# mit-han-lab/distrifuser

Hardware: NVIDIA H100
Metric: SDXL 50-step latency (ms/image) (lower is better)
Workload: dtype f16

## Files before the change

distrifuser_b200/_lib.py:

```python
from __future__ import annotations

import ctypes as C
import os

HERE = os.path.dirname(os.path.abspath(__file__))
LIB_PATH = os.environ.get("DF_LIB_PATH") or os.path.join(HERE, "libdistrifuser_b200.so")

NBANKS = 3
MAX_WORLD = 8
IPC_HANDLE_BYTES = 64
TENSORMAP_BYTES = 128
ZERO_CONV_MAX_PROBLEMS = 13

EXPORTS = (
    "df_last_error", "df_version", "df_device_sm_count", "df_symm_alloc", "df_symm_open", "df_symm_close",
    "df_symm_free", "df_step_begin", "df_slot_publish", "df_slot_wait", "df_groupnorm_scratch_bytes",
    "df_groupnorm_fwd", "df_groupnorm_halo_fwd", "df_groupnorm_fwd_weighted", "df_groupnorm_halo_fwd_weighted", "df_halo_push",
    "df_halo_assemble", "df_attn_make_kvmaps", "df_attn_workspace_bytes", "df_attn_fwd", "df_attn_make_kvmaps_ragged",
    "df_attn_workspace_bytes_ragged", "df_attn_fwd_ragged",
    "df_output_gather", "df_output_gather_2d", "df_geglu", "df_add_layernorm", "df_bias_residual_add", "df_linear_supported", "df_linear_geglu_block", "df_linear_fwd",
    "df_controlnet_zero_convs",
)


class DfComm(C.Structure):
    _fields_ = [("base", C.c_void_p * MAX_WORLD), ("flags", C.c_void_p * MAX_WORLD), ("clock", C.c_void_p),
                ("tickets", C.c_void_p), ("bank_stride", C.c_uint64), ("spin_timeout_ns", C.c_uint64), ("world", C.c_int32),
                ("rank", C.c_int32)]


_lib = None


def lib():
    global _lib
    if _lib is None:
        if not os.path.exists(LIB_PATH):
            raise RuntimeError(
                f"{LIB_PATH} is missing: build it with `python -m distrifuser_b200.build` "
                "(distrifuser_b200 has no fallback path; the CUDA extension is the product)")
        L = C.CDLL(LIB_PATH)
        vp, u64, i32, u32, i64, f32 = C.c_void_p, C.c_uint64, C.c_int, C.c_uint32, C.c_int64, C.c_float
        L.df_last_error.restype = C.c_char_p
        L.df_version.restype = i32
        L.df_device_sm_count.argtypes = [C.POINTER(i32)]
        L.df_symm_alloc.argtypes = [C.c_size_t, C.POINTER(vp), vp]
        L.df_symm_open.argtypes = [vp, C.POINTER(vp)]
        L.df_symm_close.argtypes = [vp]
        L.df_symm_free.argtypes = [vp]
        L.df_step_begin.argtypes = [vp, i32, vp]
        L.df_slot_publish.argtypes = [DfComm, vp, u64, u64, u64, u64, u64, i32, u32, i32, vp]
        L.df_slot_wait.argtypes = [DfComm, i32, u32, vp]
        L.df_groupnorm_scratch_bytes.argtypes = [i32, i32, i32, i32, i32]
        L.df_groupnorm_scratch_bytes.restype = C.c_size_t
        L.df_groupnorm_fwd.argtypes = [DfComm, vp, vp, i64, vp, vp, vp, i32, i32, i32, i32, i32, f32, i32, i32, i32, i32, i32,
                                       u64, u64, u32, vp, vp]
        L.df_groupnorm_halo_fwd.argtypes = [DfComm, vp, vp, i64, vp, vp, vp, i32, i32, i32, i32, i32, f32, i32, i32, i32, i32, i32,
                                            u64, u64, u32, vp, i32, u64, u64, i32, i32, i32, i32, vp]
        i32p = C.POINTER(C.c_int32)
        L.df_groupnorm_fwd_weighted.argtypes = [DfComm, vp, vp, i64, vp, vp, vp, i32, i32, i32, i32, i32, f32, i32, i32, i32, i32,
                                                i32, u64, u64, u32, i32p, vp, vp]
        L.df_groupnorm_halo_fwd_weighted.argtypes = [DfComm, vp, vp, i64, vp, vp, vp, i32, i32, i32, i32, i32, f32, i32, i32, i32,
                                                     i32, i32, u64, u64, u32, i32p, vp, i32, u64, u64, i32, i32, i32, i32, vp]
        L.df_attn_make_kvmaps_ragged.argtypes = [DfComm, u64, u64, i32, i32p, i32, i32, vp, vp]
        L.df_attn_workspace_bytes_ragged.argtypes = [i32, i32, i32p, i32, i32, i32]
        L.df_attn_workspace_bytes_ragged.restype = C.c_size_t
        L.df_attn_fwd_ragged.argtypes = [DfComm, vp, vp, vp, vp, i32, i32, i32p, i32, i32, i64, i64, i64, i32, i32, i32p, i32,
                                         i32, f32, vp, C.c_size_t, vp]
        L.df_halo_push.argtypes = [DfComm, vp, i32, i32, i32, i32, i32, u64, u64, i32, i32, vp]
        L.df_halo_assemble.argtypes = [DfComm, vp, vp, i32, i32, i32, i32, i32, u64, u64, i32, i32, i32, vp]
        L.df_attn_make_kvmaps.argtypes = [DfComm, u64, u64, i32, i32, i32, i32, vp, vp]
        L.df_attn_workspace_bytes.argtypes = [i32, i32, i32, i32, i32, i32]
        L.df_attn_workspace_bytes.restype = C.c_size_t
        L.df_attn_fwd.argtypes = [DfComm, vp, vp, vp, vp, i32, i32, i32, i32, i32, i64, i64, i64, i32, i32,
                                  C.POINTER(C.c_int32), i32, i32, f32, vp, C.c_size_t, vp]
        L.df_geglu.argtypes = [vp, vp, i64, i32, i64, i64, vp]
        L.df_add_layernorm.argtypes = [vp, vp, vp, vp, vp, vp, i64, i32, f32, vp]
        L.df_bias_residual_add.argtypes = [vp, vp, vp, vp, i64, i32, vp]
        L.df_linear_supported.argtypes = [i64, i32, i32, i32]
        L.df_linear_geglu_block.argtypes = [i64, i32, i32]
        L.df_linear_fwd.argtypes = [DfComm, vp, vp, vp, vp, vp, i64, i32, i32, i64, i64, i64, i64, i32, i32, i32, i32, i32, u32, u64,
                                    u64, i32, vp]
        L.df_controlnet_zero_convs.argtypes = [i32, C.POINTER(vp), C.POINTER(vp), C.POINTER(vp), C.POINTER(vp),
                                               C.POINTER(i64), C.POINTER(C.c_int32), C.POINTER(C.c_int32), vp, i32, vp]
        L.df_output_gather.argtypes = [DfComm, vp, vp, i32, i32, i32, i32, i32, i32, i32, i32, i32, u64, vp]
        L.df_output_gather_2d.argtypes = [DfComm, vp, vp, i32, i32, i32, i32, i32, i32, i32, i32, i32, i32, i32, u64, vp]
        for name in EXPORTS:
            getattr(L, name)
        _lib = L
    return _lib


KERNELS_PER_CALL = {"df_groupnorm_fwd": 1, "df_groupnorm_halo_fwd": 1, "df_attn_fwd": 1, "df_groupnorm_fwd_weighted": 1,
                    "df_groupnorm_halo_fwd_weighted": 1, "df_attn_fwd_ragged": 1, "df_halo_push": 1, "df_halo_assemble": 1,
                    "df_slot_publish": 1, "df_slot_wait": 1, "df_step_begin": 1, "df_output_gather": 2, "df_output_gather_2d": 2, "df_geglu": 1, "df_add_layernorm": 1, "df_bias_residual_add": 1,
                    "df_linear_fwd": 1, "df_controlnet_zero_convs": 1}
LAUNCHES = {"total": 0}
PROFILE = None


def check(rc: int, what: str = ""):
    LAUNCHES["total"] += KERNELS_PER_CALL.get(what, 0)
    if rc != 0:
        raise RuntimeError(f"distrifuser_b200 {what} failed ({rc}): {lib().df_last_error().decode()}")


def int32_array(values) -> C.Array:
    values = list(values)
    assert len(values) <= MAX_WORLD
    return (C.c_int32 * MAX_WORLD)(*values)


def null_comm() -> DfComm:
    c = DfComm()
    c.world, c.rank, c.bank_stride = 1, 0, 0
    return c
```

distrifuser_b200/csrc/linear.cu:

```cuda
#include <math.h>
#include <string.h>

#include "tc_ptx.cuh"

using namespace df;
using namespace df::tc;

namespace {

constexpr int BM = 128;
constexpr int BK = 64;
constexpr int NCONSUMER_WARPS = 8;
constexpr int NCONSUMERS = 32 * NCONSUMER_WARPS;
constexpr int NTHREADS = NCONSUMERS + 128;
constexpr int NEPILOGUE = 96;
constexpr int NTHREADS_ZC = NCONSUMERS + 32;
constexpr int CONSUMER_REGS = 208, WG2_REGS = 88;
constexpr uint32_t A_BYTES = BM * BK * 2;

template <int BN> struct Stages { static constexpr int value = BN == 256 ? 3 : 5; };

template <int BN>
struct __align__(1024) SmemT {
  __half a[Stages<BN>::value][BM * BK];
  __half b[Stages<BN>::value][BN * BK];
  uint64_t full[Stages<BN>::value], empty[Stages<BN>::value];
};

template <int BN> __host__ __device__ constexpr int stage_pitch() { return BN + 8; }

template <int BN>
struct __align__(1024) LinearSmem {
  SmemT<BN> ring;
  __half stg[BM * stage_pitch<BN>()];
  uint64_t stg_full, stg_empty;
};

enum { EPI_PLAIN = 0, EPI_GEGLU = 1 };

struct LinearArgs {
  const __half* bias;
  const __half* residual;
  __half* out;
  int64_t M;
  int N, K;
  int64_t ldr, ldo;
  int tiles_m, tiles_n;
  int publish;
  int pub_col0, pub_cols;
  int idx;
  uint32_t peer_mask;
  uint64_t tensor_off, slot_bytes;
  df_comm_t comm;
};

__device__ __forceinline__ float gelu_erf(float x) {
  const float z = fabsf(x) * 0.70710678118654752f;
  const float t = __fdividef(1.f, fmaf(0.3275911f, z, 1.f));
  float p = fmaf(1.061405429f, t, -1.453152027f);
  p = fmaf(p, t, 1.421413741f);
  p = fmaf(p, t, -0.284496736f);
  p = fmaf(p, t, 0.254829592f);
  const float e = p * t * __expf(-z * z);
  const float phi = x >= 0.f ? 1.f - 0.5f * e : 0.5f * e;
  return x * phi;
}

__device__ __forceinline__ float2 ld_h2f(const __half* p) { return __half22float2(*reinterpret_cast<const __half2*>(p)); }

__device__ __forceinline__ void stmatrix_x4(uint32_t addr, uint32_t r0, uint32_t r1, uint32_t r2, uint32_t r3) {
  asm volatile("stmatrix.sync.aligned.m8n8.x4.shared.b16 [%0], {%1, %2, %3, %4};" ::"r"(addr), "r"(r0), "r"(r1), "r"(r2), "r"(r3)
               : "memory");
}

union H8 {
  uint4 u;
  __half2 h[4];
};

template <int BN>
__device__ __forceinline__ void wgmma_tile(float* acc, uint64_t a_desc, uint64_t b_desc, uint32_t accumulate) {
  if constexpr (BN == 256) wgmma_ss_n256(acc, a_desc, b_desc, accumulate);
  else wgmma_ss_n160(acc, a_desc, b_desc, accumulate);
}

template <int BN>
__device__ __forceinline__ void load_tile(SmemT<BN>& sm, const void* tm_a, const void* tm_w, int tm, int tn, int kblocks,
                                          uint32_t& stage, uint32_t& phase) {
  constexpr int STAGES = Stages<BN>::value;
  constexpr uint32_t B_BYTES = BN * BK * 2;
  for (int kb = 0; kb < kblocks; ++kb) {
    mbar_wait(&sm.empty[stage], phase ^ 1u);
    mbar_expect_tx(&sm.full[stage], A_BYTES + B_BYTES);
    tma_load_2d(sm.a[stage], tm_a, &sm.full[stage], kb * BK, tm * BM);
    tma_load_2d(sm.b[stage], tm_w, &sm.full[stage], kb * BK, tn * BN);
    if (++stage == STAGES) { stage = 0; phase ^= 1u; }
  }
}

template <int BN>
__device__ __forceinline__ void mma_tile(SmemT<BN>& sm, float* acc, int wg, int lane, int kblocks, uint32_t& stage,
                                         uint32_t& phase) {
  constexpr int STAGES = Stages<BN>::value;
  fence_regs<BN / 2>(acc);
  uint32_t prev = 0;
  for (int kb = 0; kb < kblocks; ++kb) {
    mbar_wait(&sm.full[stage], phase);
    const uint32_t a_addr = smem_u32(sm.a[stage]) + wg * 64 * 128, b_addr = smem_u32(sm.b[stage]);
    wgmma_fence();
#pragma unroll
    for (int kk = 0; kk < BK / 16; ++kk)
      wgmma_tile<BN>(acc, smem_desc(a_addr + kk * 32, 16, 1024), smem_desc(b_addr + kk * 32, 16, 1024), (kb | kk) > 0);
    wgmma_commit();
    wgmma_wait<1>();
    if (kb > 0 && lane == 0) mbar_arrive(&sm.empty[prev]);
    prev = stage;
    if (++stage == STAGES) { stage = 0; phase ^= 1u; }
  }
  wgmma_wait<0>();
  fence_regs<BN / 2>(acc);
  if (lane == 0) mbar_arrive(&sm.empty[prev]);
}

template <int EPI, int BN>
__global__ void __launch_bounds__(NTHREADS, 1)
linear_kernel(const __grid_constant__ CUtensorMap tm_a, const __grid_constant__ CUtensorMap tm_w, LinearArgs p) {
  static_assert(BN % 32 == 0 && BN <= 256 && (BN * BK * 2) % 1024 == 0, "tile shape");
  constexpr int STAGES = Stages<BN>::value;
  constexpr int SP = stage_pitch<BN>();
  using Smem = LinearSmem<BN>;
  extern __shared__ __align__(1024) uint8_t smem_raw[];
  Smem& sm = *reinterpret_cast<Smem*>(smem_raw);
  if ((smem_u32(smem_raw) & 1023u) != 0) __trap();
  const int warp = threadIdx.x >> 5, lane = threadIdx.x & 31;
  const int ntiles = p.tiles_m * p.tiles_n;
  const int kblocks = p.K / BK;

  if (threadIdx.x == 0) {
    for (int s = 0; s < STAGES; ++s) { mbar_init(&sm.ring.full[s], 1); mbar_init(&sm.ring.empty[s], NCONSUMER_WARPS); }
    mbar_init(&sm.stg_full, NCONSUMERS);
    mbar_init(&sm.stg_empty, NEPILOGUE);
    asm volatile("fence.mbarrier_init.release.cluster;" ::: "memory");
  }
  __syncthreads();

  if (warp < NCONSUMER_WARPS) {
    setmaxnreg_inc<CONSUMER_REGS>();
    const int wg = warp >> 2;
    const int c4 = lane & 3;
    const int mrow = wg * 64 + (warp & 3) * 16 + ((lane >> 3) & 1) * 8 + (lane & 7);
    const uint32_t st_addr = smem_u32(sm.stg) + (uint32_t)(mrow * SP + (lane >> 4) * 8) * 2u;
    uint32_t stage = 0, phase = 0, sphase = 0;
    float acc[BN / 2];
    for (int tile = blockIdx.x; tile < ntiles; tile += gridDim.x) {
      const int tn = tile / p.tiles_m;
      __half2 bias2[BN / 8];
#pragma unroll
      for (int i = 0; i < BN / 8; ++i) {
        const int col = tn * BN + 8 * i + 2 * c4;
        bias2[i] = p.bias && col < p.N ? *reinterpret_cast<const __half2*>(p.bias + col) : __float2half2_rn(0.f);
      }
      mma_tile<BN>(sm.ring, acc, wg, lane, kblocks, stage, phase);
      mbar_wait(&sm.stg_empty, sphase ^ 1u);
#pragma unroll
      for (int j = 0; j < BN / 16; ++j) {
        uint32_t r[4];
#pragma unroll
        for (int q = 0; q < 2; ++q) {
          const int i = 2 * j + q;
          const float2 bb = __half22float2(bias2[i]);
          r[2 * q] = pack_h2(acc[4 * i] + bb.x, acc[4 * i + 1] + bb.y);
          r[2 * q + 1] = pack_h2(acc[4 * i + 2] + bb.x, acc[4 * i + 3] + bb.y);
        }
        stmatrix_x4(st_addr + j * 32, r[0], r[1], r[2], r[3]);
      }
      mbar_arrive(&sm.stg_full);
      sphase ^= 1u;
    }
  } else {
    setmaxnreg_dec<WG2_REGS>();
    if (warp == NCONSUMER_WARPS) {
      if (lane == 0) {
        prefetch_tmap(&tm_a);
        prefetch_tmap(&tm_w);
        uint32_t stage = 0, phase = 0;
        for (int tile = blockIdx.x; tile < ntiles; tile += gridDim.x)
          load_tile<BN>(sm.ring, &tm_a, &tm_w, tile % p.tiles_m, tile / p.tiles_m, kblocks, stage, phase);
      }
    } else {
      const int et = threadIdx.x - (NCONSUMERS + 32);
      uint32_t pub_epoch = 0;
      if (p.publish) pub_epoch = p.comm.clock[0];
      uint32_t sphase = 0;
      for (int tile = blockIdx.x; tile < ntiles; tile += gridDim.x) {
        const int tm = tile % p.tiles_m, tn = tile / p.tiles_m;
        mbar_wait(&sm.stg_full, sphase);
        if (EPI == EPI_GEGLU) {
          constexpr int CH = BN / 16;
          for (int v = et; v < BM * CH; v += NEPILOGUE) {
            const int r = v / CH, c = v % CH;
            const int64_t grow = (int64_t)tm * BM + r;
            if (grow >= p.M) continue;
            H8 hv, gv, o;
            hv.u = *reinterpret_cast<const uint4*>(sm.stg + r * SP + 8 * c);
            gv.u = *reinterpret_cast<const uint4*>(sm.stg + r * SP + 8 * (c + CH));
#pragma unroll
            for (int k = 0; k < 4; ++k) {
              const float2 hf = __half22float2(hv.h[k]), gf = __half22float2(gv.h[k]);
              o.h[k] = __floats2half2_rn(hf.x * gelu_erf(gf.x), hf.y * gelu_erf(gf.y));
            }
            *reinterpret_cast<uint4*>(p.out + grow * p.ldo + tn * (BN / 2) + 8 * c) = o.u;
          }
        } else {
          constexpr int CH = BN / 8;
#pragma unroll 4
          for (int v = et; v < BM * CH; v += NEPILOGUE) {
            const int r = v / CH, c = v % CH;
            const int64_t grow = (int64_t)tm * BM + r;
            const int col = tn * BN + 8 * c;
            if (grow >= p.M || col >= p.N) continue;
            H8 o;
            o.u = *reinterpret_cast<const uint4*>(sm.stg + r * SP + 8 * c);
            if (p.residual) {
              H8 rv;
              rv.u = __ldg(reinterpret_cast<const uint4*>(p.residual + grow * p.ldr + col));
#pragma unroll
              for (int k = 0; k < 4; ++k) o.h[k] = __hadd2(o.h[k], rv.h[k]);
            }
            *reinterpret_cast<uint4*>(p.out + grow * p.ldo + col) = o.u;
            if (p.publish && col >= p.pub_col0) {
              const uint64_t off = slot_offset(p.comm, pub_epoch, p.tensor_off, p.slot_bytes, p.comm.rank) +
                                   ((uint64_t)grow * p.pub_cols + (col - p.pub_col0)) * 2;
              for (int q = 0; q < p.comm.world; ++q)
                if (p.peer_mask >> q & 1) *reinterpret_cast<uint4*>((char*)p.comm.base[q] + off) = o.u;
            }
          }
        }
        mbar_arrive(&sm.stg_empty);
        sphase ^= 1u;
      }
    }
  }
  if (p.publish) signal_when_last(p.comm, &p.comm.tickets[p.idx], gridDim.x, p.idx, p.peer_mask, p.comm.clock[0]);
}

int make_map2d(CUtensorMap* m, const void* base, int64_t rows, int K, int64_t pitch, int box_rows) {
  EncodeTiledFn enc = tensor_map_encoder();
  DF_REQUIRE(enc != nullptr, "cuTensorMapEncodeTiled is not available from this driver");
  cuuint64_t dims[2] = {(cuuint64_t)K, (cuuint64_t)rows};
  cuuint64_t strides[1] = {(cuuint64_t)pitch * 2};
  cuuint32_t box[2] = {BK, (cuuint32_t)box_rows};
  cuuint32_t estr[2] = {1, 1};
  CUresult r = enc(m, CU_TENSOR_MAP_DATA_TYPE_FLOAT16, 2, const_cast<void*>(base), dims, strides, box, estr,
                   CU_TENSOR_MAP_INTERLEAVE_NONE, CU_TENSOR_MAP_SWIZZLE_128B, CU_TENSOR_MAP_L2_PROMOTION_L2_256B,
                   CU_TENSOR_MAP_FLOAT_OOB_FILL_NONE);
  DF_REQUIRE(r == CUDA_SUCCESS, "cuTensorMapEncodeTiled failed (%d): base=%p rows=%lld K=%d pitch=%lld", (int)r, base,
             (long long)rows, K, (long long)pitch);
  return 0;
}

template <int EPI, int BN>
int launch_linear(const CUtensorMap& ta, const CUtensorMap& tw, const LinearArgs& args, int ctas, cudaStream_t st) {
  static bool attr_set = false;
  if (!attr_set) {
    DF_CHECK_CUDA(cudaFuncSetAttribute(linear_kernel<EPI, BN>, cudaFuncAttributeMaxDynamicSharedMemorySize, (int)sizeof(LinearSmem<BN>)));
    attr_set = true;
  }
  linear_kernel<EPI, BN><<<ctas, NTHREADS, sizeof(LinearSmem<BN>), st>>>(ta, tw, args);
  DF_CHECK_LAUNCH();
  return 0;
}

double tile_cost(int64_t M, int N, int bn, int ctas_avail) {
  const long long tm = (M + BM - 1) / BM, tn = (N + bn - 1) / bn, tiles = tm * tn;
  const long long rounds = (tiles + ctas_avail - 1) / ctas_avail;
  return (double)rounds * (bn + 64);
}

}

namespace {
int pick_bn(int64_t M, int N, int epilogue, int cap) {
  const bool ok160 = epilogue == EPI_PLAIN || N % 160 == 0, ok256 = epilogue == EPI_PLAIN || N % 256 == 0;
  if (!ok256) return ok160 ? 160 : 0;
  if (ok160 && tile_cost(M, N, 160, cap) < 0.97 * tile_cost(M, N, 256, cap)) return 160;
  return 256;
}
}

extern "C" int df_linear_supported(int64_t M, int N, int K, int epilogue) {
  if (M < 1 || N < 8 || N % 8 != 0 || K < BK || K % BK != 0) return 0;
  if (epilogue == EPI_GEGLU && pick_bn(M, N, epilogue, sm_count()) == 0) return 0;
  return 1;
}

extern "C" int df_linear_geglu_block(int64_t M, int N, int K) {
  (void)K;
  const int bn = pick_bn(M, N, EPI_GEGLU, sm_count());
  return bn / 2;
}

extern "C" int df_linear_fwd(df_comm_t comm, const void* a, const void* w, const void* bias, const void* residual, void* out,
                             int64_t M, int N, int K, int64_t lda, int64_t ldw, int64_t ldr, int64_t ldo, int epilogue,
                             int geglu_block, int publish, int pub_col0, int idx, uint32_t peer_mask, uint64_t tensor_off,
                             uint64_t slot_bytes, int max_ctas, void* stream) {
  DF_REQUIRE(epilogue == EPI_PLAIN || epilogue == EPI_GEGLU, "df_linear_fwd: unknown epilogue %d", epilogue);
  DF_REQUIRE(df_linear_supported(M, N, K, epilogue), "df_linear_fwd: unsupported shape M=%lld N=%d K=%d (N %% 8, K %% 64%s)",
             (long long)M, N, K, epilogue == EPI_GEGLU ? ", GEGLU: N % 256" : "");
  DF_REQUIRE(((uintptr_t)a % 16) == 0 && ((uintptr_t)w % 16) == 0 && ((uintptr_t)out % 16) == 0 && ((uintptr_t)bias % 16) == 0 &&
                 ((uintptr_t)residual % 16) == 0 && lda % 8 == 0 && ldw % 8 == 0 && ldo % 8 == 0 && ldr % 8 == 0,
             "df_linear_fwd: operands must be 16-byte aligned with pitches multiple of 8");
  DF_REQUIRE(!(publish && epilogue != EPI_PLAIN), "df_linear_fwd: publication is a plain-epilogue feature");
  LinearArgs args;
  memset(&args, 0, sizeof(args));
  args.bias = (const __half*)bias; args.residual = (const __half*)residual; args.out = (__half*)out;
  args.M = M; args.N = N; args.K = K; args.ldr = ldr; args.ldo = ldo;
  const int sms = sm_count();
  const int cap = max_ctas > 0 ? max_ctas : sms;
  int bn = pick_bn(M, N, epilogue, epilogue == EPI_GEGLU ? sms : cap);
  if (epilogue == EPI_GEGLU && geglu_block > 0) {
    DF_REQUIRE(geglu_block == 80 || geglu_block == 128, "df_linear_fwd: geglu_block must be 80 or 128");
    bn = 2 * geglu_block;
    DF_REQUIRE(N % bn == 0, "df_linear_fwd: interleave block %d does not tile N=%d", geglu_block, N);
  }
  args.tiles_m = (int)((M + BM - 1) / BM);
  args.tiles_n = (N + bn - 1) / bn;
  args.publish = publish && peer_mask != 0;
  args.comm = comm;
  if (args.publish) {
    DF_REQUIRE(pub_col0 >= 0 && pub_col0 < N && pub_col0 % 8 == 0, "df_linear_fwd: bad pub_col0");
    DF_REQUIRE(tensor_off % 16 == 0 && slot_bytes % 16 == 0, "df_linear_fwd: slots must be 16-byte aligned");
    args.pub_col0 = pub_col0; args.pub_cols = N - pub_col0; args.idx = idx; args.peer_mask = peer_mask;
    args.tensor_off = tensor_off; args.slot_bytes = slot_bytes;
    DF_REQUIRE((uint64_t)M * args.pub_cols * 2 <= slot_bytes, "df_linear_fwd: published columns larger than the slot");
  }
  int ctas = args.tiles_m * args.tiles_n;
  if (ctas > cap) ctas = cap;
  if (ctas < 1) ctas = 1;
  CUtensorMap ta, tw;
  if (int rc = make_map2d(&ta, a, M, K, lda, BM)) return rc;
  if (int rc = make_map2d(&tw, w, N, K, ldw, bn)) return rc;
  cudaStream_t st = (cudaStream_t)stream;
  if (epilogue == EPI_GEGLU) {
    if (bn == 160) return launch_linear<EPI_GEGLU, 160>(ta, tw, args, ctas, st);
    return launch_linear<EPI_GEGLU, 256>(ta, tw, args, ctas, st);
  }
  if (bn == 160) return launch_linear<EPI_PLAIN, 160>(ta, tw, args, ctas, st);
  return launch_linear<EPI_PLAIN, 256>(ta, tw, args, ctas, st);
}

namespace {
constexpr int ZC_BN = 160;

struct ZeroConvProblem {
  const __half* bias;
  __half* out;
  int M, N, tiles_m, tile0, kblocks;
};

struct ZeroConvArgs {
  CUtensorMap a[DF_ZERO_CONV_MAX_PROBLEMS], w[DF_ZERO_CONV_MAX_PROBLEMS];
  ZeroConvProblem p[DF_ZERO_CONV_MAX_PROBLEMS];
  const float* scale;
  int nproblems, ntiles;
};
static_assert(sizeof(ZeroConvArgs) <= 4096, "the problem list must fit the 4 KiB kernel parameter space");

__device__ __forceinline__ int zc_problem(const ZeroConvArgs& z, int tile) {
  int q = 0;
  while (q + 1 < z.nproblems && tile >= z.p[q + 1].tile0) ++q;
  return q;
}

__global__ void __launch_bounds__(NTHREADS_ZC, 1) zero_conv_kernel(const __grid_constant__ ZeroConvArgs z) {
  constexpr int BN = ZC_BN;
  constexpr int STAGES = Stages<BN>::value;
  using Smem = SmemT<BN>;
  extern __shared__ __align__(1024) uint8_t smem_raw[];
  Smem& sm = *reinterpret_cast<Smem*>(smem_raw);
  if ((smem_u32(smem_raw) & 1023u) != 0) __trap();
  const int warp = threadIdx.x >> 5, lane = threadIdx.x & 31;

  if (threadIdx.x == 0) {
    for (int s = 0; s < STAGES; ++s) { mbar_init(&sm.full[s], 1); mbar_init(&sm.empty[s], NCONSUMER_WARPS); }
    asm volatile("fence.mbarrier_init.release.cluster;" ::: "memory");
  }
  __syncthreads();

  if (warp == NCONSUMER_WARPS) {
    if (lane == 0) {
      uint32_t stage = 0, phase = 0;
      for (int tile = blockIdx.x; tile < z.ntiles; tile += gridDim.x) {
        const int q = zc_problem(z, tile);
        const ZeroConvProblem& p = z.p[q];
        const int t = tile - p.tile0;
        load_tile<BN>(sm, &z.a[q], &z.w[q], t % p.tiles_m, t / p.tiles_m, p.kblocks, stage, phase);
      }
    }
  } else {
    const int wg = warp >> 2;
    const int c4 = lane & 3;
    const int rloc = wg * 64 + (warp & 3) * 16 + (lane >> 2);
    const float scale = *z.scale;
    uint32_t stage = 0, phase = 0;
    float acc[BN / 2];
    for (int tile = blockIdx.x; tile < z.ntiles; tile += gridDim.x) {
      const ZeroConvProblem& p = z.p[zc_problem(z, tile)];
      const int t = tile - p.tile0;
      const int tm = t % p.tiles_m, tn = t / p.tiles_m;
      mma_tile<BN>(sm, acc, wg, lane, p.kblocks, stage, phase);
#pragma unroll
      for (int h = 0; h < 2; ++h) {
        const int64_t grow = (int64_t)tm * BM + rloc + 8 * h;
        if (grow >= p.M) continue;
        const int col0 = tn * BN;
        __half* dst = p.out + grow * p.N + col0;
#pragma unroll
        for (int i = 0; i < BN / 8; ++i) {
          const int c = 8 * i + 2 * c4;
          const int col = col0 + c;
          if (col >= p.N) continue;
          float2 f = make_float2(acc[4 * i + 2 * h], acc[4 * i + 2 * h + 1]);
          if (p.bias) { const float2 bb = ld_h2f(p.bias + col); f.x += bb.x; f.y += bb.y; }
          const float2 r = __half22float2(__floats2half2_rn(f.x, f.y));
          *reinterpret_cast<__half2*>(dst + c) = __floats2half2_rn(r.x * scale, r.y * scale);
        }
      }
    }
  }
}
}

extern "C" int df_controlnet_zero_convs(int nproblems, const void* const* x_host, const void* const* w_host,
                                        const void* const* bias_host, void* const* out_host, const int64_t* m_host,
                                        const int32_t* n_host, const int32_t* k_host, const float* scale, int max_ctas,
                                        void* stream) {
  DF_REQUIRE(nproblems >= 1 && nproblems <= DF_ZERO_CONV_MAX_PROBLEMS, "df_controlnet_zero_convs: %d problems (1..%d)",
             nproblems, DF_ZERO_CONV_MAX_PROBLEMS);
  DF_REQUIRE(x_host && w_host && out_host && m_host && n_host && k_host && scale, "df_controlnet_zero_convs: null argument");
  DF_REQUIRE(((uintptr_t)scale % 4) == 0, "df_controlnet_zero_convs: scale must be a 4-byte aligned fp32");
  ZeroConvArgs z;
  memset(&z, 0, sizeof(z));
  int ntiles = 0;
  for (int i = 0; i < nproblems; ++i) {
    const int64_t M = m_host[i];
    const int N = n_host[i], K = k_host[i];
    const void* bias = bias_host ? bias_host[i] : nullptr;
    DF_REQUIRE(M >= 1 && M <= INT32_MAX && N >= 8 && N % 8 == 0 && K >= 8 && K % 8 == 0,
               "df_controlnet_zero_convs: problem %d has unsupported shape M=%lld N=%d K=%d (N %% 8, K %% 8)", i,
               (long long)M, N, K);
    DF_REQUIRE(x_host[i] && w_host[i] && out_host[i] && ((uintptr_t)x_host[i] % 16) == 0 &&
                   ((uintptr_t)w_host[i] % 16) == 0 && ((uintptr_t)out_host[i] % 16) == 0 && ((uintptr_t)bias % 16) == 0,
               "df_controlnet_zero_convs: problem %d: operands must be non-null and 16-byte aligned", i);
    if (int rc = make_map2d(&z.a[i], x_host[i], M, K, K, BM)) return rc;
    if (int rc = make_map2d(&z.w[i], w_host[i], N, K, K, ZC_BN)) return rc;
    ZeroConvProblem& p = z.p[i];
    p.bias = (const __half*)bias; p.out = (__half*)out_host[i];
    p.M = (int)M; p.N = N; p.kblocks = (K + BK - 1) / BK;
    p.tiles_m = (int)((M + BM - 1) / BM);
    p.tile0 = ntiles;
    const int64_t t = (int64_t)p.tiles_m * ((N + ZC_BN - 1) / ZC_BN);
    DF_REQUIRE(ntiles + t <= INT32_MAX, "df_controlnet_zero_convs: too many tiles");
    ntiles += (int)t;
  }
  z.scale = scale; z.nproblems = nproblems; z.ntiles = ntiles;
  const int cap = max_ctas > 0 ? max_ctas : sm_count();
  const int ctas = ntiles < cap ? ntiles : cap;
  static bool attr_set = false;
  if (!attr_set) {
    DF_CHECK_CUDA(cudaFuncSetAttribute(zero_conv_kernel, cudaFuncAttributeMaxDynamicSharedMemorySize, (int)sizeof(SmemT<ZC_BN>)));
    attr_set = true;
  }
  zero_conv_kernel<<<ctas, NTHREADS_ZC, sizeof(SmemT<ZC_BN>), (cudaStream_t)stream>>>(z);
  DF_CHECK_LAUNCH();
  return 0;
}
```

distrifuser_b200/csrc/tc_ptx.cuh:

```cuda
#pragma once
#include <cuda.h>

#include "common.cuh"

namespace df {
namespace tc {

__device__ __forceinline__ uint32_t smem_u32(const void* p) { return (uint32_t)__cvta_generic_to_shared(p); }

__device__ __forceinline__ void mbar_init(uint64_t* bar, uint32_t count) {
  asm volatile("mbarrier.init.shared::cta.b64 [%0], %1;" ::"r"(smem_u32(bar)), "r"(count));
}
__device__ __forceinline__ void mbar_expect_tx(uint64_t* bar, uint32_t bytes) {
  asm volatile("mbarrier.arrive.expect_tx.shared::cta.b64 _, [%0], %1;" ::"r"(smem_u32(bar)), "r"(bytes) : "memory");
}
__device__ __forceinline__ void mbar_arrive(uint32_t bar_addr) {
  asm volatile("mbarrier.arrive.shared::cta.b64 _, [%0];" ::"r"(bar_addr) : "memory");
}
__device__ __forceinline__ void mbar_arrive(uint64_t* bar) { mbar_arrive(smem_u32(bar)); }
constexpr uint32_t kTryWaitHintNs = 200000u;
__device__ __forceinline__ bool mbar_try(uint32_t bar_addr, uint32_t parity) {
  uint32_t ok;
  asm volatile(
      "{\n\t.reg .pred p;\n\t"
      "mbarrier.try_wait.parity.shared::cta.b64 p, [%1], %2, %3;\n\t"
      "selp.u32 %0, 1, 0, p;\n\t}"
      : "=r"(ok)
      : "r"(bar_addr), "r"(parity), "r"(kTryWaitHintNs)
      : "memory");
  return ok != 0;
}
__device__ __forceinline__ bool mbar_try(uint64_t* bar, uint32_t parity) { return mbar_try(smem_u32(bar), parity); }
__device__ __forceinline__ void mbar_wait(uint32_t bar, uint32_t parity) {
  if (mbar_try(bar, parity)) return;
  uint32_t polls = 0;
  uint64_t t0 = 0;
  while (!mbar_try(bar, parity)) {
    if ((++polls & 0x3FFu) == 0) {
      const uint64_t now = globaltimer_ns();
      if (t0 == 0) t0 = now;
      else if (now - t0 > 10000000000ull) {
#ifdef DF_MBAR_DEBUG
        printf("distrifuser_b200: mbarrier timeout (block %d,%d,%d thread %d bar@%u parity %u)\n", blockIdx.x, blockIdx.y, blockIdx.z,
               threadIdx.x, bar, parity);
#endif
        __trap();
      }
    }
  }
}

__device__ __forceinline__ void mbar_wait(uint64_t* bar, uint32_t parity) { mbar_wait(smem_u32(bar), parity); }

__device__ __forceinline__ void tma_load_4d(void* dst, const void* tmap, uint64_t* bar, int c0, int c1, int c2, int c3) {
  asm volatile(
      "cp.async.bulk.tensor.4d.shared::cluster.global.mbarrier::complete_tx::bytes [%0], [%1, {%3, %4, %5, %6}], [%2];"
      ::"r"(smem_u32(dst)), "l"((uint64_t)tmap), "r"(smem_u32(bar)), "r"(c0), "r"(c1), "r"(c2), "r"(c3)
      : "memory");
}
__device__ __forceinline__ void tma_load_2d(void* dst, const void* tmap, uint64_t* bar, int c0, int c1) {
  asm volatile(
      "cp.async.bulk.tensor.2d.shared::cluster.global.mbarrier::complete_tx::bytes [%0], [%1, {%3, %4}], [%2];"
      ::"r"(smem_u32(dst)), "l"((uint64_t)tmap), "r"(smem_u32(bar)), "r"(c0), "r"(c1)
      : "memory");
}
__device__ __forceinline__ void prefetch_tmap(const void* tmap) {
  asm volatile("prefetch.tensormap [%0];" ::"l"((uint64_t)tmap) : "memory");
}

__device__ __forceinline__ uint64_t smem_desc(uint32_t addr, uint32_t lbo_bytes, uint32_t sbo_bytes) {
  return (uint64_t)((addr & 0x3FFFFu) >> 4) | ((uint64_t)((lbo_bytes >> 4) & 0x3FFFu) << 16) |
         ((uint64_t)((sbo_bytes >> 4) & 0x3FFFu) << 32) | (1ull << 62);
}
__device__ __forceinline__ void wgmma_fence() { asm volatile("wgmma.fence.sync.aligned;" ::: "memory"); }
__device__ __forceinline__ void wgmma_commit() { asm volatile("wgmma.commit_group.sync.aligned;" ::: "memory"); }
template <int N>
__device__ __forceinline__ void wgmma_wait() { asm volatile("wgmma.wait_group.sync.aligned %0;" ::"n"(N) : "memory"); }
template <int N>
__device__ __forceinline__ void setmaxnreg_dec() { asm volatile("setmaxnreg.dec.sync.aligned.u32 %0;" ::"n"(N)); }
template <int N>
__device__ __forceinline__ void setmaxnreg_inc() { asm volatile("setmaxnreg.inc.sync.aligned.u32 %0;" ::"n"(N)); }
template <int ID, int COUNT>
__device__ __forceinline__ void named_bar_sync() { asm volatile("bar.sync %0, %1;" ::"n"(ID), "n"(COUNT) : "memory"); }
template <int ID, int COUNT>
__device__ __forceinline__ void named_bar_arrive() { asm volatile("bar.arrive %0, %1;" ::"n"(ID), "n"(COUNT) : "memory"); }
template <int N>
__device__ __forceinline__ void fence_regs(float* d) {
#pragma unroll
  for (int i = 0; i < N; ++i) asm volatile("" : "+f"(d[i])::"memory");
}

__device__ __forceinline__ void wgmma_ss_n64(float* d, uint64_t a_desc, uint64_t b_desc, uint32_t accumulate) {
  asm volatile(
      "{\n\t.reg .pred p;\n\tsetp.ne.b32 p, %34, 0;\n\t"
      "wgmma.mma_async.sync.aligned.m64n64k16.f32.f16.f16 {%0, %1, %2, %3, %4, %5, %6, %7, %8, %9, %10, %11, %12, %13, %14, %15, %16, %17, %18, %19, %20, %21, %22, %23, %24, %25, %26, %27, %28, %29, %30, %31}, %32, %33, p, 1, 1, 0, 0;\n\t}"
      : "+f"(d[0]), "+f"(d[1]), "+f"(d[2]), "+f"(d[3]), "+f"(d[4]), "+f"(d[5]), "+f"(d[6]), "+f"(d[7]), "+f"(d[8]), "+f"(d[9]), "+f"(d[10]), "+f"(d[11]), "+f"(d[12]), "+f"(d[13]), "+f"(d[14]), "+f"(d[15]), "+f"(d[16]), "+f"(d[17]), "+f"(d[18]), "+f"(d[19]), "+f"(d[20]), "+f"(d[21]), "+f"(d[22]), "+f"(d[23]), "+f"(d[24]), "+f"(d[25]), "+f"(d[26]), "+f"(d[27]), "+f"(d[28]), "+f"(d[29]), "+f"(d[30]), "+f"(d[31])
      : "l"(a_desc), "l"(b_desc), "r"(accumulate));
}
__device__ __forceinline__ void wgmma_ss_n128(float* d, uint64_t a_desc, uint64_t b_desc, uint32_t accumulate) {
  asm volatile(
      "{\n\t.reg .pred p;\n\tsetp.ne.b32 p, %66, 0;\n\t"
      "wgmma.mma_async.sync.aligned.m64n128k16.f32.f16.f16 {%0, %1, %2, %3, %4, %5, %6, %7, %8, %9, %10, %11, %12, %13, %14, %15, %16, %17, %18, %19, %20, %21, %22, %23, %24, %25, %26, %27, %28, %29, %30, %31, %32, %33, %34, %35, %36, %37, %38, %39, %40, %41, %42, %43, %44, %45, %46, %47, %48, %49, %50, %51, %52, %53, %54, %55, %56, %57, %58, %59, %60, %61, %62, %63}, %64, %65, p, 1, 1, 0, 0;\n\t}"
      : "+f"(d[0]), "+f"(d[1]), "+f"(d[2]), "+f"(d[3]), "+f"(d[4]), "+f"(d[5]), "+f"(d[6]), "+f"(d[7]), "+f"(d[8]), "+f"(d[9]), "+f"(d[10]), "+f"(d[11]), "+f"(d[12]), "+f"(d[13]), "+f"(d[14]), "+f"(d[15]), "+f"(d[16]), "+f"(d[17]), "+f"(d[18]), "+f"(d[19]), "+f"(d[20]), "+f"(d[21]), "+f"(d[22]), "+f"(d[23]), "+f"(d[24]), "+f"(d[25]), "+f"(d[26]), "+f"(d[27]), "+f"(d[28]), "+f"(d[29]), "+f"(d[30]), "+f"(d[31]), "+f"(d[32]), "+f"(d[33]), "+f"(d[34]), "+f"(d[35]), "+f"(d[36]), "+f"(d[37]), "+f"(d[38]), "+f"(d[39]), "+f"(d[40]), "+f"(d[41]), "+f"(d[42]), "+f"(d[43]), "+f"(d[44]), "+f"(d[45]), "+f"(d[46]), "+f"(d[47]), "+f"(d[48]), "+f"(d[49]), "+f"(d[50]), "+f"(d[51]), "+f"(d[52]), "+f"(d[53]), "+f"(d[54]), "+f"(d[55]), "+f"(d[56]), "+f"(d[57]), "+f"(d[58]), "+f"(d[59]), "+f"(d[60]), "+f"(d[61]), "+f"(d[62]), "+f"(d[63])
      : "l"(a_desc), "l"(b_desc), "r"(accumulate));
}

__device__ __forceinline__ void wgmma_ss_n160(float* d, uint64_t a_desc, uint64_t b_desc, uint32_t accumulate) {
  asm volatile(
      "{\n\t.reg .pred p;\n\tsetp.ne.b32 p, %82, 0;\n\t"
      "wgmma.mma_async.sync.aligned.m64n160k16.f32.f16.f16 {%0, %1, %2, %3, %4, %5, %6, %7, %8, %9, %10, %11, %12, %13, %14, %15, %16, %17, %18, %19, %20, %21, %22, %23, %24, %25, %26, %27, %28, %29, %30, %31, %32, %33, %34, %35, %36, %37, %38, %39, %40, %41, %42, %43, %44, %45, %46, %47, %48, %49, %50, %51, %52, %53, %54, %55, %56, %57, %58, %59, %60, %61, %62, %63, %64, %65, %66, %67, %68, %69, %70, %71, %72, %73, %74, %75, %76, %77, %78, %79}, %80, %81, p, 1, 1, 0, 0;\n\t}"
      : "+f"(d[0]), "+f"(d[1]), "+f"(d[2]), "+f"(d[3]), "+f"(d[4]), "+f"(d[5]), "+f"(d[6]), "+f"(d[7]), "+f"(d[8]), "+f"(d[9]), "+f"(d[10]), "+f"(d[11]), "+f"(d[12]), "+f"(d[13]), "+f"(d[14]), "+f"(d[15]), "+f"(d[16]), "+f"(d[17]), "+f"(d[18]), "+f"(d[19]), "+f"(d[20]), "+f"(d[21]), "+f"(d[22]), "+f"(d[23]), "+f"(d[24]), "+f"(d[25]), "+f"(d[26]), "+f"(d[27]), "+f"(d[28]), "+f"(d[29]), "+f"(d[30]), "+f"(d[31]), "+f"(d[32]), "+f"(d[33]), "+f"(d[34]), "+f"(d[35]), "+f"(d[36]), "+f"(d[37]), "+f"(d[38]), "+f"(d[39]), "+f"(d[40]), "+f"(d[41]), "+f"(d[42]), "+f"(d[43]), "+f"(d[44]), "+f"(d[45]), "+f"(d[46]), "+f"(d[47]), "+f"(d[48]), "+f"(d[49]), "+f"(d[50]), "+f"(d[51]), "+f"(d[52]), "+f"(d[53]), "+f"(d[54]), "+f"(d[55]), "+f"(d[56]), "+f"(d[57]), "+f"(d[58]), "+f"(d[59]), "+f"(d[60]), "+f"(d[61]), "+f"(d[62]), "+f"(d[63]), "+f"(d[64]), "+f"(d[65]), "+f"(d[66]), "+f"(d[67]), "+f"(d[68]), "+f"(d[69]), "+f"(d[70]), "+f"(d[71]), "+f"(d[72]), "+f"(d[73]), "+f"(d[74]), "+f"(d[75]), "+f"(d[76]), "+f"(d[77]), "+f"(d[78]), "+f"(d[79])
      : "l"(a_desc), "l"(b_desc), "r"(accumulate));
}

__device__ __forceinline__ void wgmma_ss_n256(float* d, uint64_t a_desc, uint64_t b_desc, uint32_t accumulate) {
  asm volatile(
      "{\n\t.reg .pred p;\n\tsetp.ne.b32 p, %130, 0;\n\t"
      "wgmma.mma_async.sync.aligned.m64n256k16.f32.f16.f16 {%0, %1, %2, %3, %4, %5, %6, %7, %8, %9, %10, %11, %12, %13, %14, %15, %16, %17, %18, %19, %20, %21, %22, %23, %24, %25, %26, %27, %28, %29, %30, %31, %32, %33, %34, %35, %36, %37, %38, %39, %40, %41, %42, %43, %44, %45, %46, %47, %48, %49, %50, %51, %52, %53, %54, %55, %56, %57, %58, %59, %60, %61, %62, %63, %64, %65, %66, %67, %68, %69, %70, %71, %72, %73, %74, %75, %76, %77, %78, %79, %80, %81, %82, %83, %84, %85, %86, %87, %88, %89, %90, %91, %92, %93, %94, %95, %96, %97, %98, %99, %100, %101, %102, %103, %104, %105, %106, %107, %108, %109, %110, %111, %112, %113, %114, %115, %116, %117, %118, %119, %120, %121, %122, %123, %124, %125, %126, %127}, %128, %129, p, 1, 1, 0, 0;\n\t}"
      : "+f"(d[0]), "+f"(d[1]), "+f"(d[2]), "+f"(d[3]), "+f"(d[4]), "+f"(d[5]), "+f"(d[6]), "+f"(d[7]), "+f"(d[8]), "+f"(d[9]), "+f"(d[10]), "+f"(d[11]), "+f"(d[12]), "+f"(d[13]), "+f"(d[14]), "+f"(d[15]), "+f"(d[16]), "+f"(d[17]), "+f"(d[18]), "+f"(d[19]), "+f"(d[20]), "+f"(d[21]), "+f"(d[22]), "+f"(d[23]), "+f"(d[24]), "+f"(d[25]), "+f"(d[26]), "+f"(d[27]), "+f"(d[28]), "+f"(d[29]), "+f"(d[30]), "+f"(d[31]), "+f"(d[32]), "+f"(d[33]), "+f"(d[34]), "+f"(d[35]), "+f"(d[36]), "+f"(d[37]), "+f"(d[38]), "+f"(d[39]), "+f"(d[40]), "+f"(d[41]), "+f"(d[42]), "+f"(d[43]), "+f"(d[44]), "+f"(d[45]), "+f"(d[46]), "+f"(d[47]), "+f"(d[48]), "+f"(d[49]), "+f"(d[50]), "+f"(d[51]), "+f"(d[52]), "+f"(d[53]), "+f"(d[54]), "+f"(d[55]), "+f"(d[56]), "+f"(d[57]), "+f"(d[58]), "+f"(d[59]), "+f"(d[60]), "+f"(d[61]), "+f"(d[62]), "+f"(d[63]), "+f"(d[64]), "+f"(d[65]), "+f"(d[66]), "+f"(d[67]), "+f"(d[68]), "+f"(d[69]), "+f"(d[70]), "+f"(d[71]), "+f"(d[72]), "+f"(d[73]), "+f"(d[74]), "+f"(d[75]), "+f"(d[76]), "+f"(d[77]), "+f"(d[78]), "+f"(d[79]), "+f"(d[80]), "+f"(d[81]), "+f"(d[82]), "+f"(d[83]), "+f"(d[84]), "+f"(d[85]), "+f"(d[86]), "+f"(d[87]), "+f"(d[88]), "+f"(d[89]), "+f"(d[90]), "+f"(d[91]), "+f"(d[92]), "+f"(d[93]), "+f"(d[94]), "+f"(d[95]), "+f"(d[96]), "+f"(d[97]), "+f"(d[98]), "+f"(d[99]), "+f"(d[100]), "+f"(d[101]), "+f"(d[102]), "+f"(d[103]), "+f"(d[104]), "+f"(d[105]), "+f"(d[106]), "+f"(d[107]), "+f"(d[108]), "+f"(d[109]), "+f"(d[110]), "+f"(d[111]), "+f"(d[112]), "+f"(d[113]), "+f"(d[114]), "+f"(d[115]), "+f"(d[116]), "+f"(d[117]), "+f"(d[118]), "+f"(d[119]), "+f"(d[120]), "+f"(d[121]), "+f"(d[122]), "+f"(d[123]), "+f"(d[124]), "+f"(d[125]), "+f"(d[126]), "+f"(d[127])
      : "l"(a_desc), "l"(b_desc), "r"(accumulate));
}

__device__ __forceinline__ void wgmma_rs_n64(float* d, const uint32_t* a, uint64_t b_desc, uint32_t accumulate) {
  asm volatile(
      "{\n\t.reg .pred p;\n\tsetp.ne.b32 p, %37, 0;\n\t"
      "wgmma.mma_async.sync.aligned.m64n64k16.f32.f16.f16 {%0, %1, %2, %3, %4, %5, %6, %7, %8, %9, %10, %11, %12, %13, %14, %15, %16, %17, %18, %19, %20, %21, %22, %23, %24, %25, %26, %27, %28, %29, %30, %31}, {%32, %33, %34, %35}, %36, p, 1, 1, 1;\n\t}"
      : "+f"(d[0]), "+f"(d[1]), "+f"(d[2]), "+f"(d[3]), "+f"(d[4]), "+f"(d[5]), "+f"(d[6]), "+f"(d[7]), "+f"(d[8]), "+f"(d[9]), "+f"(d[10]), "+f"(d[11]), "+f"(d[12]), "+f"(d[13]), "+f"(d[14]), "+f"(d[15]), "+f"(d[16]), "+f"(d[17]), "+f"(d[18]), "+f"(d[19]), "+f"(d[20]), "+f"(d[21]), "+f"(d[22]), "+f"(d[23]), "+f"(d[24]), "+f"(d[25]), "+f"(d[26]), "+f"(d[27]), "+f"(d[28]), "+f"(d[29]), "+f"(d[30]), "+f"(d[31])
      : "r"(a[0]), "r"(a[1]), "r"(a[2]), "r"(a[3]), "l"(b_desc), "r"(accumulate));
}


__device__ __forceinline__ float ex2(float x) {
  float y;
  asm("ex2.approx.ftz.f32 %0, %1;" : "=f"(y) : "f"(x));
  return y;
}
__device__ __forceinline__ float ex2_poly(float x) {
  x = fmaxf(x, -127.f);
  const float r = __fadd_rd(x, 12582912.f);
  const float f = x - (r - 12582912.f);
  float q = fmaf(f, 0.077119089663028717041015625f, 0.227564394474029541015625f);
  q = fmaf(q, f, 0.695146143436431884765625f);
  q = fmaf(q, f, 1.f);
  return __int_as_float(__float_as_int(q) + (__float_as_int(r) << 23));
}
__device__ __forceinline__ uint32_t pack_h2(float lo, float hi) {
  __half2 h = __floats2half2_rn(lo, hi);
  return *reinterpret_cast<uint32_t*>(&h);
}


}
}
```

distrifuser_b200/modules/pp/attn.py:

```python
import ctypes as C

import torch
from torch import nn
from torch.nn import functional as F

from ... import _lib
from ...utils import DistriConfig
from ..base_module import BaseModule, nvtx_range


_WORKSPACES: dict = {}


def _shared_workspace(device, nbytes: int) -> torch.Tensor:
    lst = _WORKSPACES.setdefault(device, [])
    if not lst or lst[-1].numel() < nbytes:
        if torch.cuda.is_current_stream_capturing():
            raise RuntimeError("attention workspace would grow during CUDA-graph capture; run one eager UNet call first")
        lst.append(torch.zeros(max(nbytes, 16 << 20), dtype=torch.uint8, device=device))
    return lst[-1]


class DistriAttentionPP(BaseModule):
    def __init__(self, module: nn.Module, distri_config: DistriConfig):
        super().__init__(module, distri_config)
        to_k, to_v = module.to_k, module.to_v
        assert isinstance(to_k, nn.Linear) and isinstance(to_v, nn.Linear)
        assert (to_k.bias is None) == (to_v.bias is None)
        assert to_k.weight.shape == to_v.weight.shape
        in_size, out_size = to_k.in_features, to_k.out_features
        to_kv = nn.Linear(in_size, out_size * 2, bias=to_k.bias is not None, device=to_k.weight.device,
                          dtype=to_k.weight.dtype)
        with torch.no_grad():
            to_kv.weight[:out_size].copy_(to_k.weight)
            to_kv.weight[out_size:].copy_(to_v.weight)
            if to_k.bias is not None:
                to_kv.bias[:out_size].copy_(to_k.bias)
                to_kv.bias[out_size:].copy_(to_v.bias)
        self.to_kv = to_kv
        self._kvmaps = None

    def _attend(self, q, kv_own, lens, own_seg, wait_flags, kind="self", scale=0.0, real_width=None):
        attn = self.module
        b, lq, Cq = q.shape
        heads = attn.heads
        d = Cq // heads
        out = torch.empty((b, lq, Cq), dtype=q.dtype, device=q.device)
        cm = self.comm_manager
        nseg = len(lens)
        if nseg > 1:
            comm, maps = cm.group, self._kvmaps.data_ptr()
        else:
            comm, maps = _lib.null_comm(), None
        seg_rank = (C.c_int32 * _lib.MAX_WORLD)(*range(_lib.MAX_WORLD))
        seg_len = _lib.int32_array(lens)
        L = _lib.lib()
        ws_bytes = L.df_attn_workspace_bytes_ragged(b, lq, seg_len, nseg, heads, d)
        ws = _shared_workspace(q.device, ws_bytes).data_ptr() if ws_bytes else None
        prof = _lib.PROFILE
        if prof is not None:
            e0, e1 = torch.cuda.Event(enable_timing=True), torch.cuda.Event(enable_timing=True)
            e0.record()
        _lib.check(L.df_attn_fwd_ragged(comm, q.data_ptr(), kv_own.data_ptr(), out.data_ptr(), maps, b, lq, seg_len,
                                        heads, d, q.stride(1), kv_own.stride(1), out.stride(1), nseg, own_seg,
                                        seg_rank, self.idx or 0, int(wait_flags), float(scale), ws, ws_bytes,
                                        torch.cuda.current_stream().cuda_stream), "df_attn_fwd_ragged")
        if prof is not None:
            e1.record()
            prof.append(dict(kernel="fmha_fwd_kernel", kind=kind,
                             flops=4.0 * b * lq * sum(lens) * (real_width or Cq),
                             bytes=2.0 * (2 * b * lq * Cq + b * sum(lens) * 2 * Cq),
                             shape=(b, lq, sum(lens), heads, d), start=e0, end=e1))
        return out

    def _project_out(self, hidden_states, residual, weight=None):
        from ... import ops
        attn = self.module
        hidden_states = ops.project("out", hidden_states, attn.to_out[0], weight)
        hidden_states = attn.to_out[1](hidden_states)
        if attn.residual_connection:
            hidden_states = hidden_states + residual
        if attn.rescale_output_factor != 1.0:
            hidden_states = hidden_states / attn.rescale_output_factor
        return hidden_states


class DistriCrossAttentionPP(DistriAttentionPP):
    def __init__(self, module: nn.Module, distri_config: DistriConfig):
        super().__init__(module, distri_config)
        self.kv_cache = None

    @nvtx_range("DistriCrossAttentionPP")
    def forward(self, hidden_states, encoder_hidden_states=None, scale: float = 1.0, *args, **kwargs):
        assert encoder_hidden_states is not None
        self._require_cuda_half(hidden_states, "DistriCrossAttentionPP")
        attn = self.module
        from ... import ops
        q = ops.project("qkv", hidden_states, attn.to_q)
        if self.counter == 0 or self.kv_cache is None:
            kv = self.to_kv(encoder_hidden_states)
            if self.kv_cache is not None and self.kv_cache.shape == kv.shape:
                self.kv_cache.copy_(kv)
            else:
                self.kv_cache = kv
        kv = self.kv_cache
        out = self._attend(q, kv, [kv.shape[1]], 0, False, kind="cross")
        out = self._project_out(out, hidden_states)
        self.counter += 1
        return out


class DistriSelfAttentionPP(DistriAttentionPP):
    def __init__(self, module: nn.Module, distri_config: DistriConfig):
        super().__init__(module, distri_config)
        self._w_qkv = None
        self._w_qkv_key = None
        self._w_out = None
        self._head_pad = 0

    def _qkv_weight(self, dtype):
        to_q, to_kv = self.module.to_q, self.to_kv
        if not (isinstance(to_q, nn.Linear) and to_q.bias is None and to_kv.bias is None and
                to_q.in_features == to_kv.in_features and to_q.out_features * 2 == to_kv.out_features and
                to_q.weight.dtype == dtype and to_kv.weight.dtype == dtype):
            return None
        wq, wkv, wo = to_q.weight, to_kv.weight, self.module.to_out[0].weight
        heads = self.module.heads
        d = to_q.out_features // heads
        pad = 64 if d < 64 else 0
        key = (wq._version, wkv._version, wo._version, wq.data_ptr(), wkv.data_ptr(), wo.data_ptr(), wq.device, dtype, pad)
        if key != self._w_qkv_key:
            if torch.cuda.is_current_stream_capturing():
                raise RuntimeError("DistriSelfAttentionPP: attention weights changed since the last eager call; run one "
                                   "eager UNet call (pipeline.prepare()) before capturing CUDA graphs")
            with torch.no_grad():
                if pad:
                    cin = wq.shape[1]
                    widen = lambda w: F.pad(w.detach().reshape(-1, heads, d, cin), (0, 0, 0, pad - d)).reshape(-1, cin)
                    self._w_qkv = torch.cat([widen(wq), widen(wkv)], 0).contiguous()
                    self._w_out = F.pad(wo.detach().reshape(wo.shape[0], heads, d), (0, pad - d)).reshape(wo.shape[0], heads * pad).contiguous()
                else:
                    self._w_qkv = torch.cat([wq.detach(), wkv.detach()], 0).contiguous()
                    self._w_out = None
            self._w_qkv_key = key
            self._head_pad = pad
        return self._w_qkv

    @nvtx_range("DistriSelfAttentionPP")
    def forward(self, hidden_states, encoder_hidden_states=None, scale: float = 1.0, *args, **kwargs):
        cfg = self.distri_config
        self._require_cuda_half(hidden_states, "DistriSelfAttentionPP")
        attn = self.module
        n, r = cfg.n_device_per_batch, cfg.split_idx()
        b, l, c = hidden_states.shape
        cm = self.comm_manager
        w_qkv = self._qkv_weight(hidden_states.dtype)
        heads = attn.heads
        d_real = c // heads
        padded = w_qkv is not None and self._head_pad != 0
        cs = heads * self._head_pad if padded else c
        lens = self.patch_rows(l) if n > 1 else [l]
        if n > 1 and self._recording() and self.idx is None:
            self.idx = cm.register_tensor((b, l, 2 * cs), hidden_states.dtype, layer_type="attn",
                                          slot_bytes=b * max(lens) * 2 * cs * hidden_states.element_size())
        live = n > 1 and self._bound()
        sync = live and (cfg.mode == "full_sync" or self._is_sync_step())
        ship = live and (sync or cfg.mode != "no_sync")
        published = False
        if w_qkv is not None:
            from ... import ops
            if not padded and ops.use_fused_linear("qkv") and ops.linear_supported(b * l, 3 * c, c):
                pub = (cm.group, c, self.idx, cm.peers_mask(), cm.tensor_off[self.idx], cm.slot_bytes[self.idx]) if ship else None
                qkv = ops.linear(hidden_states, w_qkv, publish=pub)
                published = ship
            else:
                qkv = F.linear(hidden_states, w_qkv)
            q, kv = qkv[..., :cs], qkv[..., cs:]
        else:
            q = attn.to_q(hidden_states)
            kv = self.to_kv(hidden_states)
        sm_scale = d_real ** -0.5 if padded else 0.0
        if not live:
            out = self._attend(q, kv, [l], 0, False, scale=sm_scale, real_width=c)
        else:
            if self._kvmaps is None:
                self._kvmaps = torch.empty(_lib.NBANKS * n * _lib.TENSORMAP_BYTES, dtype=torch.uint8, device=q.device)
                _lib.check(_lib.lib().df_attn_make_kvmaps_ragged(cm.group, cm.tensor_off[self.idx], cm.slot_bytes[self.idx], b,
                                                                 _lib.int32_array(lens), heads, cs // heads,
                                                                 self._kvmaps.data_ptr(), torch.cuda.current_stream().cuda_stream),
                           "df_attn_make_kvmaps_ragged")
            if ship and not published:
                cm.enqueue(self.idx, kv, async_stream=not sync)
            out = self._attend(q, kv, lens, r, True, scale=sm_scale, real_width=c)
        out = self._project_out(out, hidden_states, self._w_out if padded else None)
        self.counter += 1
        return out
```

distrifuser_b200/ops.py:

```python
import os as _os

import torch

from . import _lib


def geglu(y: torch.Tensor) -> torch.Tensor:
    assert y.is_cuda and y.dtype == torch.float16 and y.stride(-1) == 1
    cols = y.shape[-1] // 2
    y2 = y.reshape(-1, 2 * cols)
    out = torch.empty((*y.shape[:-1], cols), dtype=y.dtype, device=y.device)
    _lib.check(_lib.lib().df_geglu(y2.data_ptr(), out.data_ptr(), y2.shape[0], cols, y2.stride(0), cols,
                                   torch.cuda.current_stream().cuda_stream), "df_geglu")
    return out


def add_layernorm(x: torch.Tensor, r: torch.Tensor | None, norm: torch.nn.LayerNorm):
    assert x.is_cuda and x.dtype == torch.float16
    C = x.shape[-1]
    x = x.contiguous()
    y = torch.empty_like(x)
    if r is not None:
        r = r.contiguous()
        s = torch.empty_like(x)
    else:
        s = x
    _lib.check(_lib.lib().df_add_layernorm(x.data_ptr(), r.data_ptr() if r is not None else None,
                                           s.data_ptr() if r is not None else None, y.data_ptr(), norm.weight.data_ptr(),
                                           norm.bias.data_ptr(), x.numel() // C, C, float(norm.eps),
                                           torch.cuda.current_stream().cuda_stream), "df_add_layernorm")
    return s, y


def conv2d_bias_residual(x: torch.Tensor, conv: torch.nn.Conv2d, padding, residual: torch.Tensor | None = None,
                         bias: torch.Tensor | None = None, fold_bias: bool = False) -> torch.Tensor:
    import torch.nn.functional as F
    b = conv.bias if bias is None else bias
    ok = (x.is_cuda and x.dtype == torch.float16 and conv.out_channels % 8 == 0 and
          x.is_contiguous(memory_format=torch.channels_last))
    if not ok:
        out = F.conv2d(x, conv.weight, None if fold_bias else b, stride=conv.stride, padding=padding)
        return out if residual is None else residual + out
    out = F.conv2d(x, conv.weight, None, stride=conv.stride, padding=padding)
    if (b is None or fold_bias) and residual is None:
        return out
    if not out.is_contiguous(memory_format=torch.channels_last):
        out = out.contiguous(memory_format=torch.channels_last)
    if b is None or fold_bias:
        return residual + out
    if residual is not None:
        assert residual.shape == out.shape and residual.dtype == out.dtype
        if not residual.is_contiguous(memory_format=torch.channels_last):
            residual = residual.contiguous(memory_format=torch.channels_last)
    n, c, h, w = out.shape
    _lib.check(_lib.lib().df_bias_residual_add(out.data_ptr(), residual.data_ptr() if residual is not None else None,
                                               b.data_ptr(), out.data_ptr(), n * h * w, c,
                                               torch.cuda.current_stream().cuda_stream), "df_bias_residual_add")
    return out



_FUSED_LINEAR = set(_os.environ.get("DF_LINEAR", "geglu").replace("all", "geglu,qkv,out,ff2,proj").split(","))


def use_fused_linear(kind: str) -> bool:
    return kind in _FUSED_LINEAR


GEGLU_BLOCK = 128


def linear_supported(M: int, N: int, K: int, geglu: bool = False) -> bool:
    return bool(_lib.lib().df_linear_supported(M, N, K, 1 if geglu else 0))


def geglu_block(M: int, two_d: int, K: int) -> int:
    if not linear_supported(M, two_d, K, geglu=True):
        return 0
    return int(_lib.lib().df_linear_geglu_block(M, two_d, K))


def geglu_interleave(weight: torch.Tensor, bias: torch.Tensor | None, block: int = GEGLU_BLOCK):
    two_d, K = weight.shape
    D = two_d // 2
    assert D % block == 0
    w = torch.stack([weight[:D].reshape(D // block, block, K), weight[D:].reshape(D // block, block, K)], 1)
    w = w.reshape(two_d, K).contiguous()
    b = None
    if bias is not None:
        b = torch.stack([bias[:D].reshape(-1, block), bias[D:].reshape(-1, block)], 1).reshape(two_d).contiguous()
    return w, b


def linear(x: torch.Tensor, weight: torch.Tensor, bias: torch.Tensor | None = None, residual: torch.Tensor | None = None,
           out: torch.Tensor | None = None, publish=None) -> torch.Tensor:
    assert x.is_cuda and x.dtype == torch.float16 and weight.dtype == torch.float16 and x.stride(-1) == 1 and weight.stride(-1) == 1
    K = x.shape[-1]
    N = weight.shape[0]
    x2 = x.reshape(-1, K)
    M = x2.shape[0]
    if out is None:
        out = torch.empty((*x.shape[:-1], N), dtype=x.dtype, device=x.device)
    o2 = out.view(-1, N)
    r2 = residual.reshape(-1, N) if residual is not None else None
    if publish is not None:
        comm, pub_col0, idx, mask, off, sb = publish
    else:
        comm, pub_col0, idx, mask, off, sb = _lib.null_comm(), 0, 0, 0, 0, 0
    _lib.check(_lib.lib().df_linear_fwd(comm, x2.data_ptr(), weight.data_ptr(), bias.data_ptr() if bias is not None else None,
                                        r2.data_ptr() if r2 is not None else None, o2.data_ptr(), M, N, K, x2.stride(0),
                                        weight.stride(0), r2.stride(0) if r2 is not None else 0, o2.stride(0), 0, 0,
                                        int(publish is not None), pub_col0, idx, mask, off, sb, 0,
                                        torch.cuda.current_stream().cuda_stream), "df_linear_fwd")
    return out


def project(kind: str, x: torch.Tensor, lin: torch.nn.Linear, weight: torch.Tensor | None = None) -> torch.Tensor:
    w = lin.weight if weight is None else weight
    K = x.shape[-1]
    if (use_fused_linear(kind) and x.is_cuda and x.dtype == torch.float16 and w.dtype == torch.float16 and
            x.stride(-1) == 1 and w.stride(-1) == 1 and getattr(lin, "lora_layer", None) is None and
            linear_supported(x.numel() // K, w.shape[0], K)):
        return linear(x, w, lin.bias)
    if weight is None:
        return lin(x)
    import torch.nn.functional as F
    return F.linear(x, weight, lin.bias)


def linear_geglu(x: torch.Tensor, w_interleaved: torch.Tensor, b_interleaved: torch.Tensor | None, block: int = GEGLU_BLOCK) -> torch.Tensor:
    assert x.is_cuda and x.dtype == torch.float16 and x.stride(-1) == 1
    K = x.shape[-1]
    N = w_interleaved.shape[0]
    x2 = x.reshape(-1, K)
    out = torch.empty((*x.shape[:-1], N // 2), dtype=x.dtype, device=x.device)
    _lib.check(_lib.lib().df_linear_fwd(_lib.null_comm(), x2.data_ptr(), w_interleaved.data_ptr(),
                                        b_interleaved.data_ptr() if b_interleaved is not None else None, None, out.data_ptr(),
                                        x2.shape[0], N, K, x2.stride(0), w_interleaved.stride(0), 0, N // 2, 1, block, 0, 0, 0, 0, 0, 0, 0,
                                        torch.cuda.current_stream().cuda_stream), "df_linear_fwd")
    return out


def controlnet_zero_convs(xs, convs, scale: torch.Tensor) -> list[torch.Tensor]:
    import ctypes as C
    n = len(xs)
    assert len(convs) == n and scale.is_cuda and scale.dtype == torch.float32 and scale.numel() == 1
    outs, xp, wp, bp, op, ms, ns, ks = [], [], [], [], [], [], [], []
    for x, conv in zip(xs, convs):
        assert x.is_cuda and x.dtype == torch.float16 and tuple(conv.kernel_size) == (1, 1)
        x = x.contiguous(memory_format=torch.channels_last)
        b, k, h, w = x.shape
        out = torch.empty((b, conv.out_channels, h, w), dtype=x.dtype, device=x.device, memory_format=torch.channels_last)
        outs.append(out)
        xp.append(x.data_ptr()); wp.append(conv.weight.data_ptr()); op.append(out.data_ptr())
        bp.append(conv.bias.data_ptr() if conv.bias is not None else None)
        ms.append(b * h * w); ns.append(conv.out_channels); ks.append(k)
    ptrs = lambda v: (C.c_void_p * n)(*v)
    _lib.check(_lib.lib().df_controlnet_zero_convs(n, ptrs(xp), ptrs(wp), ptrs(bp), ptrs(op), (C.c_int64 * n)(*ms),
                                                   (C.c_int32 * n)(*ns), (C.c_int32 * n)(*ks), scale.data_ptr(), 0,
                                                   torch.cuda.current_stream().cuda_stream), "df_controlnet_zero_convs")
    return outs
```

include/distrifuser_b200.h:

```cpp
#ifndef DISTRIFUSER_B200_H
#define DISTRIFUSER_B200_H

#include <stddef.h>
#include <stdint.h>

#ifdef __cplusplus
extern "C" {
#endif

#define DF_NBANKS 3
#define DF_MAX_WORLD 8
#define DF_IPC_HANDLE_BYTES 64
#define DF_TENSORMAP_BYTES 128
#define DF_ZERO_CONV_MAX_PROBLEMS 13

const char* df_last_error(void);
int df_version(void);
int df_device_sm_count(int* out);

int df_symm_alloc(size_t bytes, void** dptr, void* ipc_handle_out_host );
int df_symm_open(const void* ipc_handle_host, void** peer_dptr);
int df_symm_close(void* peer_dptr);
int df_symm_free(void* dptr);

typedef struct {
  void* base[DF_MAX_WORLD];
  uint32_t* flags[DF_MAX_WORLD];
  uint32_t* clock;
  uint32_t* tickets;
  uint64_t bank_stride;
  uint64_t spin_timeout_ns;
  int32_t world;
  int32_t rank;
} df_comm_t;

int df_step_begin(uint32_t* clock, int kind, void* stream);

int df_slot_publish(df_comm_t comm, const void* src, uint64_t rows, uint64_t row_bytes, uint64_t src_pitch,
                    uint64_t tensor_off, uint64_t slot_bytes, int idx, uint32_t peer_mask, int num_ctas,
                    void* stream);

int df_slot_wait(df_comm_t comm, int idx, uint32_t src_mask, void* stream);

size_t df_groupnorm_scratch_bytes(int b, int groups, int h, int w, int C);
int df_groupnorm_fwd(df_comm_t comm, const void* x, const void* addend, int64_t addend_pitch, void* y, const void* gamma, const void* beta,
                     int b, int h, int w, int C, int groups, float eps, int mode, int bessel,
                     int neg_var_fallback, int fuse_silu, int idx, uint64_t tensor_off, uint64_t slot_bytes,
                     uint32_t group_mask, void* scratch, void* stream);

int df_groupnorm_halo_fwd(df_comm_t comm, const void* x, const void* addend, int64_t addend_pitch, void* y_padded, const void* gamma, const void* beta,
                          int b, int h, int w, int C, int groups, float eps, int mode, int bessel, int neg_var_fallback,
                          int fuse_silu, int idx, uint64_t tensor_off, uint64_t slot_bytes, uint32_t group_mask, void* scratch,
                          int halo_idx, uint64_t halo_off, uint64_t halo_slot_bytes, int up_rank, int down_rank, int push,
                          int wait_flags, void* stream);

int df_groupnorm_fwd_weighted(df_comm_t comm, const void* x, const void* addend, int64_t addend_pitch, void* y, const void* gamma,
                              const void* beta, int b, int h, int w, int C, int groups, float eps, int mode, int bessel,
                              int neg_var_fallback, int fuse_silu, int idx, uint64_t tensor_off, uint64_t slot_bytes,
                              uint32_t group_mask, const int32_t* src_weight_host , void* scratch, void* stream);
int df_groupnorm_halo_fwd_weighted(df_comm_t comm, const void* x, const void* addend, int64_t addend_pitch, void* y_padded,
                                   const void* gamma, const void* beta, int b, int h, int w, int C, int groups, float eps, int mode,
                                   int bessel, int neg_var_fallback, int fuse_silu, int idx, uint64_t tensor_off,
                                   uint64_t slot_bytes, uint32_t group_mask, const int32_t* src_weight_host ,
                                   void* scratch, int halo_idx, uint64_t halo_off, uint64_t halo_slot_bytes, int up_rank,
                                   int down_rank, int push, int wait_flags, void* stream);

int df_halo_push(df_comm_t comm, const void* x, int b, int h, int w, int C, int idx, uint64_t tensor_off,
                 uint64_t slot_bytes, int up_rank, int down_rank, void* stream);
int df_halo_assemble(df_comm_t comm, const void* x, void* xp, int b, int h, int w, int C, int idx,
                     uint64_t tensor_off, uint64_t slot_bytes, int up_rank, int down_rank, int wait_flags,
                     void* stream);

int df_attn_make_kvmaps(df_comm_t comm, uint64_t tensor_off, uint64_t slot_bytes, int b, int lseg, int heads,
                        int d, void* maps_out , void* stream);
size_t df_attn_workspace_bytes(int b, int lq, int lseg, int nseg, int heads, int d);
int df_attn_fwd(df_comm_t comm, const void* q, const void* kv_own, void* out, const void* kvmaps,
                int b, int lq, int lseg, int heads, int d, int64_t q_pitch, int64_t kv_pitch, int64_t o_pitch,
                int nseg, int own_seg, const int32_t* seg_rank_host, int idx, int wait_flags, float scale,
                void* workspace, size_t workspace_bytes, void* stream);
int df_attn_make_kvmaps_ragged(df_comm_t comm, uint64_t tensor_off, uint64_t slot_bytes, int b, const int32_t* seg_len_host,
                               int heads, int d, void* maps_out , void* stream);
size_t df_attn_workspace_bytes_ragged(int b, int lq, const int32_t* seg_len_host, int nseg, int heads, int d);
int df_attn_fwd_ragged(df_comm_t comm, const void* q, const void* kv_own, void* out, const void* kvmaps,
                       int b, int lq, const int32_t* seg_len_host, int heads, int d, int64_t q_pitch, int64_t kv_pitch,
                       int64_t o_pitch, int nseg, int own_seg, const int32_t* seg_rank_host, int idx, int wait_flags, float scale,
                       void* workspace, size_t workspace_bytes, void* stream);

int df_output_gather(df_comm_t comm, const void* strip, void* out, int B, int C, int H, int W, int bs, int hs,
                     int batch0, int row0, int idx, uint64_t tensor_off, void* stream);

int df_output_gather_2d(df_comm_t comm, const void* strip, void* out, int B, int C, int H, int W, int bs, int hs, int ws,
                        int batch0, int row0, int col0, int idx, uint64_t tensor_off, void* stream);

int df_geglu(const void* in, void* out, int64_t rows, int cols, int64_t in_pitch, int64_t out_pitch, void* stream);

int df_bias_residual_add(const void* a, const void* residual , const void* bias, void* out, int64_t rows, int C,
                         void* stream);

int df_add_layernorm(const void* x, const void* r, void* s_out, void* y, const void* gamma, const void* beta,
                     int64_t rows, int C, float eps, void* stream);

int df_linear_supported(int64_t M, int N, int K, int epilogue);
int df_linear_geglu_block(int64_t M, int N, int K);
int df_linear_fwd(df_comm_t comm, const void* a, const void* w, const void* bias, const void* residual, void* out,
                  int64_t M, int N, int K, int64_t lda, int64_t ldw, int64_t ldr, int64_t ldo, int epilogue,
                  int geglu_block, int publish, int pub_col0, int idx, uint32_t peer_mask, uint64_t tensor_off,
                  uint64_t slot_bytes, int max_ctas, void* stream);

int df_controlnet_zero_convs(int nproblems, const void* const* x_host, const void* const* w_host, const void* const* bias_host,
                             void* const* out_host, const int64_t* m_host, const int32_t* n_host, const int32_t* k_host,
                             const float* scale, int max_ctas, void* stream);

#ifdef __cplusplus
}
#endif
#endif
```

Before: 1521.

## Fuse cross-attention Q projection and softmax attention into the linear GEMM kernel

Adds a cross-attention epilogue to the warp-specialized linear kernel. After the Q projection tile is computed, the kernel adds the bias and, for each 64-wide head, runs QK^T, softmax and PV in registers against the cached text K/V (at most 80 tokens), with K/V loaded by TMA into the ring stages. This removes the separate Q projection kernel, the round trip of Q through global memory and the separate attention launch. In exchange it adds N=192/128 tile variants, higher register pressure, and a new code path limited to head_dim 64 and at most 80 KV tokens.

```diff
diff --git a/distrifuser_b200/_lib.py b/distrifuser_b200/_lib.py
--- a/distrifuser_b200/_lib.py
+++ b/distrifuser_b200/_lib.py
@@ -19,7 +19,7 @@
     "df_halo_assemble", "df_attn_make_kvmaps", "df_attn_workspace_bytes", "df_attn_fwd", "df_attn_make_kvmaps_ragged",
     "df_attn_workspace_bytes_ragged", "df_attn_fwd_ragged",
     "df_output_gather", "df_output_gather_2d", "df_geglu", "df_add_layernorm", "df_bias_residual_add", "df_linear_supported", "df_linear_geglu_block", "df_linear_fwd",
-    "df_controlnet_zero_convs",
+    "df_linear_cross_attn_supported", "df_linear_cross_attn_fwd", "df_controlnet_zero_convs",
 )
 
 
@@ -81,6 +81,8 @@
         L.df_linear_geglu_block.argtypes = [i64, i32, i32]
         L.df_linear_fwd.argtypes = [DfComm, vp, vp, vp, vp, vp, i64, i32, i32, i64, i64, i64, i64, i32, i32, i32, i32, i32, u32, u64,
                                     u64, i32, vp]
+        L.df_linear_cross_attn_supported.argtypes = [i32, i32, i32, i32, i32, i32]
+        L.df_linear_cross_attn_fwd.argtypes = [vp, vp, vp, vp, vp, i32, i32, i32, i32, i32, i32, i64, i64, f32, i32, vp]
         L.df_controlnet_zero_convs.argtypes = [i32, C.POINTER(vp), C.POINTER(vp), C.POINTER(vp), C.POINTER(vp),
                                                C.POINTER(i64), C.POINTER(C.c_int32), C.POINTER(C.c_int32), vp, i32, vp]
         L.df_output_gather.argtypes = [DfComm, vp, vp, i32, i32, i32, i32, i32, i32, i32, i32, i32, u64, vp]
@@ -94,7 +96,7 @@
 KERNELS_PER_CALL = {"df_groupnorm_fwd": 1, "df_groupnorm_halo_fwd": 1, "df_attn_fwd": 1, "df_groupnorm_fwd_weighted": 1,
                     "df_groupnorm_halo_fwd_weighted": 1, "df_attn_fwd_ragged": 1, "df_halo_push": 1, "df_halo_assemble": 1,
                     "df_slot_publish": 1, "df_slot_wait": 1, "df_step_begin": 1, "df_output_gather": 2, "df_output_gather_2d": 2, "df_geglu": 1, "df_add_layernorm": 1, "df_bias_residual_add": 1,
-                    "df_linear_fwd": 1, "df_controlnet_zero_convs": 1}
+                    "df_linear_fwd": 1, "df_linear_cross_attn_fwd": 1, "df_controlnet_zero_convs": 1}
 LAUNCHES = {"total": 0}
 PROFILE = None
 
diff --git a/distrifuser_b200/csrc/linear.cu b/distrifuser_b200/csrc/linear.cu
--- a/distrifuser_b200/csrc/linear.cu
+++ b/distrifuser_b200/csrc/linear.cu
@@ -18,7 +18,7 @@
 constexpr int CONSUMER_REGS = 208, WG2_REGS = 88;
 constexpr uint32_t A_BYTES = BM * BK * 2;
 
-template <int BN> struct Stages { static constexpr int value = BN == 256 ? 3 : 5; };
+template <int BN> struct Stages { static constexpr int value = BN == 256 ? 3 : BN == 192 ? 4 : 5; };
 
 template <int BN>
 struct __align__(1024) SmemT {
@@ -36,7 +36,11 @@
   uint64_t stg_full, stg_empty;
 };
 
-enum { EPI_PLAIN = 0, EPI_GEGLU = 1 };
+enum { EPI_PLAIN = 0, EPI_GEGLU = 1, EPI_CROSS = 2 };
+
+constexpr int HEAD_D = 64;
+constexpr int LKV_ROWS = 80;
+constexpr uint32_t KV_BYTES = LKV_ROWS * HEAD_D * 2;
 
 struct LinearArgs {
   const __half* bias;
@@ -52,6 +56,8 @@
   uint32_t peer_mask;
   uint64_t tensor_off, slot_bytes;
   df_comm_t comm;
+  int L, mt, lkv;
+  float scale_log2;
 };
 
 __device__ __forceinline__ float gelu_erf(float x) {
@@ -81,18 +87,21 @@
 template <int BN>
 __device__ __forceinline__ void wgmma_tile(float* acc, uint64_t a_desc, uint64_t b_desc, uint32_t accumulate) {
   if constexpr (BN == 256) wgmma_ss_n256(acc, a_desc, b_desc, accumulate);
-  else wgmma_ss_n160(acc, a_desc, b_desc, accumulate);
+  else if constexpr (BN == 192) wgmma_ss_n192(acc, a_desc, b_desc, accumulate);
+  else if constexpr (BN == 160) wgmma_ss_n160(acc, a_desc, b_desc, accumulate);
+  else wgmma_ss_n128(acc, a_desc, b_desc, accumulate);
 }
 
 template <int BN>
-__device__ __forceinline__ void load_tile(SmemT<BN>& sm, const void* tm_a, const void* tm_w, int tm, int tn, int kblocks,
-                                          uint32_t& stage, uint32_t& phase) {
+__device__ __forceinline__ void load_tile(SmemT<BN>& sm, const void* tm_a, const void* tm_w, int a_row, int a_bat, int tn,
+                                          int kblocks, uint32_t& stage, uint32_t& phase) {
   constexpr int STAGES = Stages<BN>::value;
   constexpr uint32_t B_BYTES = BN * BK * 2;
   for (int kb = 0; kb < kblocks; ++kb) {
     mbar_wait(&sm.empty[stage], phase ^ 1u);
     mbar_expect_tx(&sm.full[stage], A_BYTES + B_BYTES);
-    tma_load_2d(sm.a[stage], tm_a, &sm.full[stage], kb * BK, tm * BM);
+    if (a_bat < 0) tma_load_2d(sm.a[stage], tm_a, &sm.full[stage], kb * BK, a_row);
+    else tma_load_3d(sm.a[stage], tm_a, &sm.full[stage], kb * BK, a_row, a_bat);
     tma_load_2d(sm.b[stage], tm_w, &sm.full[stage], kb * BK, tn * BN);
     if (++stage == STAGES) { stage = 0; phase ^= 1u; }
   }
@@ -122,10 +131,115 @@
   if (lane == 0) mbar_arrive(&sm.empty[prev]);
 }
 
+template <int BN>
+__device__ __forceinline__ void cross_attend(SmemT<BN>& sm, float* acc, const __half2* bias2, uint32_t st_addr, int lane,
+                                             int lkv, float scale_log2, uint32_t& stage, uint32_t& phase) {
+  constexpr int STAGES = Stages<BN>::value;
+  constexpr int NH = BN / HEAD_D;
+  const int c4 = lane & 3;
+  uint32_t qf[BN / 4];
+#pragma unroll
+  for (int i = 0; i < BN / 8; ++i) {
+    const float2 bb = __half22float2(bias2[i]);
+    qf[2 * i] = pack_h2(acc[4 * i] + bb.x, acc[4 * i + 1] + bb.y);
+    qf[2 * i + 1] = pack_h2(acc[4 * i + 2] + bb.x, acc[4 * i + 3] + bb.y);
+  }
+  uint32_t hs[NH], hp[NH];
+#pragma unroll
+  for (int h = 0; h < NH; ++h) {
+    hs[h] = stage; hp[h] = phase;
+    if (++stage == STAGES) { stage = 0; phase ^= 1u; }
+  }
+  auto k_addr = [&](int h) { return BN == 256 ? smem_u32(sm.b[hs[h]]) : smem_u32(sm.a[hs[h]]); };
+  auto v_addr = [&](int h) { return BN == 256 ? smem_u32(sm.b[hs[h]]) + KV_BYTES : smem_u32(sm.b[hs[h]]); };
+  constexpr bool S_IN_ACC = LKV_ROWS <= BN / 2, O_IN_ACC = LKV_ROWS + HEAD_D / 2 <= BN / 2;
+  float s_own[S_IN_ACC ? 1 : LKV_ROWS], o_own[O_IN_ACC ? 1 : HEAD_D / 2];
+  float* const s_buf = S_IN_ACC ? acc : s_own;
+  float* s[2] = {s_buf, s_buf + LKV_ROWS / 2};
+  auto issue_s = [&](int h) {
+    mbar_wait(&sm.full[hs[h]], hp[h]);
+    wgmma_fence();
+#pragma unroll
+    for (int kk = 0; kk < HEAD_D / 16; ++kk)
+      wgmma_rs_n80(s[h & 1], qf + 16 * h + 4 * kk, smem_desc(k_addr(h) + kk * 32, 16, 1024), kk > 0);
+    wgmma_commit();
+  };
+  issue_s(0);
+#pragma unroll
+  for (int h = 0; h < NH; ++h) {
+    float* S = s[h & 1];
+    if (h + 1 < NH) {
+      issue_s(h + 1);
+      wgmma_wait<1>();
+    } else {
+      wgmma_wait<0>();
+    }
+    fence_regs<LKV_ROWS / 2>(S);
+    auto sv = [&](int i, int k) {
+      const float x = S[4 * i + k];
+      return 8 * i + 2 * c4 + (k & 1) >= lkv ? -INFINITY : x;
+    };
+    float mA0 = -INFINITY, mA1 = -INFINITY, mB0 = -INFINITY, mB1 = -INFINITY;
+#pragma unroll
+    for (int i = 0; i < LKV_ROWS / 8; i += 2) {
+      mA0 = fmaxf(mA0, fmaxf(sv(i, 0), sv(i, 1)));
+      mB0 = fmaxf(mB0, fmaxf(sv(i, 2), sv(i, 3)));
+      mA1 = fmaxf(mA1, fmaxf(sv(i + 1, 0), sv(i + 1, 1)));
+      mB1 = fmaxf(mB1, fmaxf(sv(i + 1, 2), sv(i + 1, 3)));
+    }
+    float mA = fmaxf(mA0, mA1), mB = fmaxf(mB0, mB1);
+    mA = fmaxf(mA, __shfl_xor_sync(0xffffffffu, mA, 1));
+    mB = fmaxf(mB, __shfl_xor_sync(0xffffffffu, mB, 1));
+    mA = fmaxf(mA, __shfl_xor_sync(0xffffffffu, mA, 2));
+    mB = fmaxf(mB, __shfl_xor_sync(0xffffffffu, mB, 2));
+    const float nA = -mA * scale_log2, nB = -mB * scale_log2;
+    float lA = 0.f, lB = 0.f;
+    uint32_t pk[LKV_ROWS / 4];
+#pragma unroll
+    for (int i = 0; i < LKV_ROWS / 8; ++i) {
+      const float p0 = ex2(fmaf(sv(i, 0), scale_log2, nA)), p1 = ex2(fmaf(sv(i, 1), scale_log2, nA));
+      const float p2 = ex2(fmaf(sv(i, 2), scale_log2, nB)), p3 = ex2(fmaf(sv(i, 3), scale_log2, nB));
+      lA += p0 + p1;
+      lB += p2 + p3;
+      pk[2 * i] = pack_h2(p0, p1);
+      pk[2 * i + 1] = pack_h2(p2, p3);
+    }
+    float* o = O_IN_ACC ? acc + LKV_ROWS : o_own;
+    wgmma_fence();
+#pragma unroll
+    for (int kk = 0; kk < LKV_ROWS / 16; ++kk)
+      wgmma_rs_n64(o, pk + 4 * kk, smem_desc(v_addr(h) + kk * 2048, KV_BYTES, 1024), kk > 0);
+    wgmma_commit();
+    lA += __shfl_xor_sync(0xffffffffu, lA, 1); lB += __shfl_xor_sync(0xffffffffu, lB, 1);
+    lA += __shfl_xor_sync(0xffffffffu, lA, 2); lB += __shfl_xor_sync(0xffffffffu, lB, 2);
+    const float invA = 1.f / lA, invB = 1.f / lB;
+    wgmma_wait<0>();
+    fence_regs<HEAD_D / 2>(o);
+    if (h + 1 < NH) fence_regs<LKV_ROWS / 2>(s[(h + 1) & 1]);
+    __syncwarp();
+    if (lane == 0) mbar_arrive(&sm.empty[hs[h]]);
+#pragma unroll
+    for (int j = 0; j < HEAD_D / 16; ++j) {
+      uint32_t r[4];
+#pragma unroll
+      for (int q = 0; q < 2; ++q) {
+        const int i = 2 * j + q;
+        r[2 * q] = pack_h2(o[4 * i] * invA, o[4 * i + 1] * invA);
+        r[2 * q + 1] = pack_h2(o[4 * i + 2] * invB, o[4 * i + 3] * invB);
+      }
+      stmatrix_x4(st_addr + (h * (HEAD_D / 16) + j) * 32, r[0], r[1], r[2], r[3]);
+    }
+  }
+}
+
 template <int EPI, int BN>
 __global__ void __launch_bounds__(NTHREADS, 1)
-linear_kernel(const __grid_constant__ CUtensorMap tm_a, const __grid_constant__ CUtensorMap tm_w, LinearArgs p) {
+linear_kernel(const __grid_constant__ CUtensorMap tm_a, const __grid_constant__ CUtensorMap tm_w,
+              const __grid_constant__ CUtensorMap tm_kv, LinearArgs p) {
   static_assert(BN % 32 == 0 && BN <= 256 && (BN * BK * 2) % 1024 == 0, "tile shape");
+  static_assert(EPI != EPI_CROSS || (BN % HEAD_D == 0 && (BN == 256 ? 2 * KV_BYTES <= BN * BK * 2
+                                                                    : KV_BYTES <= A_BYTES && KV_BYTES <= BN * BK * 2)),
+                "cross-attention: whole heads per tile, K and V of a head in one stage");
   constexpr int STAGES = Stages<BN>::value;
   constexpr int SP = stage_pitch<BN>();
   using Smem = LinearSmem<BN>;
@@ -162,17 +276,21 @@
       }
       mma_tile<BN>(sm.ring, acc, wg, lane, kblocks, stage, phase);
       mbar_wait(&sm.stg_empty, sphase ^ 1u);
-#pragma unroll
-      for (int j = 0; j < BN / 16; ++j) {
-        uint32_t r[4];
-#pragma unroll
-        for (int q = 0; q < 2; ++q) {
-          const int i = 2 * j + q;
-          const float2 bb = __half22float2(bias2[i]);
-          r[2 * q] = pack_h2(acc[4 * i] + bb.x, acc[4 * i + 1] + bb.y);
-          r[2 * q + 1] = pack_h2(acc[4 * i + 2] + bb.x, acc[4 * i + 3] + bb.y);
+      if constexpr (EPI == EPI_CROSS) {
+        cross_attend<BN>(sm.ring, acc, bias2, st_addr, lane, p.lkv, p.scale_log2, stage, phase);
+      } else {
+#pragma unroll
+        for (int j = 0; j < BN / 16; ++j) {
+          uint32_t r[4];
+#pragma unroll
+          for (int q = 0; q < 2; ++q) {
+            const int i = 2 * j + q;
+            const float2 bb = __half22float2(bias2[i]);
+            r[2 * q] = pack_h2(acc[4 * i] + bb.x, acc[4 * i + 1] + bb.y);
+            r[2 * q + 1] = pack_h2(acc[4 * i + 2] + bb.x, acc[4 * i + 3] + bb.y);
+          }
+          stmatrix_x4(st_addr + j * 32, r[0], r[1], r[2], r[3]);
         }
-        stmatrix_x4(st_addr + j * 32, r[0], r[1], r[2], r[3]);
       }
       mbar_arrive(&sm.stg_full);
       sphase ^= 1u;
@@ -183,9 +301,28 @@
       if (lane == 0) {
         prefetch_tmap(&tm_a);
         prefetch_tmap(&tm_w);
+        if (EPI == EPI_CROSS) prefetch_tmap(&tm_kv);
         uint32_t stage = 0, phase = 0;
-        for (int tile = blockIdx.x; tile < ntiles; tile += gridDim.x)
-          load_tile<BN>(sm.ring, &tm_a, &tm_w, tile % p.tiles_m, tile / p.tiles_m, kblocks, stage, phase);
+        for (int tile = blockIdx.x; tile < ntiles; tile += gridDim.x) {
+          const int tm = tile % p.tiles_m, tn = tile / p.tiles_m;
+          if constexpr (EPI == EPI_CROSS) {
+            const int bat = tm / p.mt;
+            load_tile<BN>(sm.ring, &tm_a, &tm_w, (tm - bat * p.mt) * BM, bat, tn, kblocks, stage, phase);
+#pragma unroll
+            for (int hh = 0; hh < BN / HEAD_D; ++hh) {
+              mbar_wait(&sm.ring.empty[stage], phase ^ 1u);
+              mbar_expect_tx(&sm.ring.full[stage], 2 * KV_BYTES);
+              __half* kdst = BN == 256 ? sm.ring.b[stage] : sm.ring.a[stage];
+              __half* vdst = BN == 256 ? sm.ring.b[stage] + LKV_ROWS * HEAD_D : sm.ring.b[stage];
+              const int c = tn * BN + hh * HEAD_D;
+              tma_load_3d(kdst, &tm_kv, &sm.ring.full[stage], c, 0, bat);
+              tma_load_3d(vdst, &tm_kv, &sm.ring.full[stage], p.N + c, 0, bat);
+              if (++stage == STAGES) { stage = 0; phase ^= 1u; }
+            }
+          } else {
+            load_tile<BN>(sm.ring, &tm_a, &tm_w, tm * BM, -1, tn, kblocks, stage, phase);
+          }
+        }
       }
     } else {
       const int et = threadIdx.x - (NCONSUMERS + 32);
@@ -194,6 +331,12 @@
       uint32_t sphase = 0;
       for (int tile = blockIdx.x; tile < ntiles; tile += gridDim.x) {
         const int tm = tile % p.tiles_m, tn = tile / p.tiles_m;
+        int64_t row0 = (int64_t)tm * BM, nrows = p.M - row0;
+        if constexpr (EPI == EPI_CROSS) {
+          const int bat = tm / p.mt, r0 = (tm - bat * p.mt) * BM;
+          row0 = (int64_t)bat * p.L + r0;
+          nrows = p.L - r0;
+        }
         mbar_wait(&sm.stg_full, sphase);
         if (EPI == EPI_GEGLU) {
           constexpr int CH = BN / 16;
@@ -216,9 +359,9 @@
 #pragma unroll 4
           for (int v = et; v < BM * CH; v += NEPILOGUE) {
             const int r = v / CH, c = v % CH;
-            const int64_t grow = (int64_t)tm * BM + r;
+            const int64_t grow = row0 + r;
             const int col = tn * BN + 8 * c;
-            if (grow >= p.M || col >= p.N) continue;
+            if (r >= nrows || col >= p.N) continue;
             H8 o;
             o.u = *reinterpret_cast<const uint4*>(sm.stg + r * SP + 8 * c);
             if (p.residual) {
@@ -259,14 +402,30 @@
   return 0;
 }
 
+int make_map3d(CUtensorMap* m, const void* base, int cols, int rows, int batch, int64_t pitch, int box_rows) {
+  EncodeTiledFn enc = tensor_map_encoder();
+  DF_REQUIRE(enc != nullptr, "cuTensorMapEncodeTiled is not available from this driver");
+  cuuint64_t dims[3] = {(cuuint64_t)cols, (cuuint64_t)rows, (cuuint64_t)batch};
+  cuuint64_t strides[2] = {(cuuint64_t)pitch * 2, (cuuint64_t)rows * pitch * 2};
+  cuuint32_t box[3] = {BK, (cuuint32_t)box_rows, 1};
+  cuuint32_t estr[3] = {1, 1, 1};
+  CUresult r = enc(m, CU_TENSOR_MAP_DATA_TYPE_FLOAT16, 3, const_cast<void*>(base), dims, strides, box, estr,
+                   CU_TENSOR_MAP_INTERLEAVE_NONE, CU_TENSOR_MAP_SWIZZLE_128B, CU_TENSOR_MAP_L2_PROMOTION_L2_256B,
+                   CU_TENSOR_MAP_FLOAT_OOB_FILL_NONE);
+  DF_REQUIRE(r == CUDA_SUCCESS, "cuTensorMapEncodeTiled failed (%d): base=%p cols=%d rows=%d batch=%d pitch=%lld", (int)r, base,
+             cols, rows, batch, (long long)pitch);
+  return 0;
+}
+
 template <int EPI, int BN>
-int launch_linear(const CUtensorMap& ta, const CUtensorMap& tw, const LinearArgs& args, int ctas, cudaStream_t st) {
+int launch_linear(const CUtensorMap& ta, const CUtensorMap& tw, const CUtensorMap& tkv, const LinearArgs& args, int ctas,
+                  cudaStream_t st) {
   static bool attr_set = false;
   if (!attr_set) {
     DF_CHECK_CUDA(cudaFuncSetAttribute(linear_kernel<EPI, BN>, cudaFuncAttributeMaxDynamicSharedMemorySize, (int)sizeof(LinearSmem<BN>)));
     attr_set = true;
   }
-  linear_kernel<EPI, BN><<<ctas, NTHREADS, sizeof(LinearSmem<BN>), st>>>(ta, tw, args);
+  linear_kernel<EPI, BN><<<ctas, NTHREADS, sizeof(LinearSmem<BN>), st>>>(ta, tw, tkv, args);
   DF_CHECK_LAUNCH();
   return 0;
 }
@@ -337,16 +496,64 @@
   int ctas = args.tiles_m * args.tiles_n;
   if (ctas > cap) ctas = cap;
   if (ctas < 1) ctas = 1;
-  CUtensorMap ta, tw;
+  CUtensorMap ta, tw, none;
+  memset(&none, 0, sizeof(none));
   if (int rc = make_map2d(&ta, a, M, K, lda, BM)) return rc;
   if (int rc = make_map2d(&tw, w, N, K, ldw, bn)) return rc;
   cudaStream_t st = (cudaStream_t)stream;
   if (epilogue == EPI_GEGLU) {
-    if (bn == 160) return launch_linear<EPI_GEGLU, 160>(ta, tw, args, ctas, st);
-    return launch_linear<EPI_GEGLU, 256>(ta, tw, args, ctas, st);
-  }
-  if (bn == 160) return launch_linear<EPI_PLAIN, 160>(ta, tw, args, ctas, st);
-  return launch_linear<EPI_PLAIN, 256>(ta, tw, args, ctas, st);
+    if (bn == 160) return launch_linear<EPI_GEGLU, 160>(ta, tw, none, args, ctas, st);
+    return launch_linear<EPI_GEGLU, 256>(ta, tw, none, args, ctas, st);
+  }
+  if (bn == 160) return launch_linear<EPI_PLAIN, 160>(ta, tw, none, args, ctas, st);
+  return launch_linear<EPI_PLAIN, 256>(ta, tw, none, args, ctas, st);
+}
+
+namespace {
+int pick_bn_cross(int64_t tiles_m, int C, int cap) {
+  int bn = 256;
+  for (int w : {192, 128})
+    if (tile_cost(tiles_m * BM, C, w, cap) < 0.97 * tile_cost(tiles_m * BM, C, bn, cap)) bn = w;
+  return bn;
+}
+}
+
+extern "C" int df_linear_cross_attn_supported(int b, int L, int C, int K, int heads, int lkv) {
+  if (b < 1 || L < 1 || heads < 1 || C != HEAD_D * heads || K < BK || K % BK != 0) return 0;
+  if (lkv < 1 || lkv > LKV_ROWS) return 0;
+  return (int64_t)b * ((L + BM - 1) / BM) * heads <= INT32_MAX;
+}
+
+extern "C" int df_linear_cross_attn_fwd(const void* x, const void* w, const void* bias, const void* kv, void* out, int b, int L,
+                                        int C, int K, int heads, int lkv, int64_t ldw, int64_t ldkv, float scale, int max_ctas,
+                                        void* stream) {
+  DF_REQUIRE(df_linear_cross_attn_supported(b, L, C, K, heads, lkv),
+             "df_linear_cross_attn_fwd: unsupported shape b=%d L=%d C=%d K=%d heads=%d lkv=%d (head width 64, "
+             "K %% 64, lkv <= 80)", b, L, C, K, heads, lkv);
+  DF_REQUIRE(x && w && kv && out && ((uintptr_t)x % 16) == 0 && ((uintptr_t)w % 16) == 0 && ((uintptr_t)kv % 16) == 0 &&
+                 ((uintptr_t)out % 16) == 0 && ((uintptr_t)bias % 16) == 0 && ldw % 8 == 0 && ldw >= K && ldkv % 8 == 0 &&
+                 ldkv >= 2 * C,
+             "df_linear_cross_attn_fwd: operands must be non-null and 16-byte aligned with pitches multiple of 8");
+  LinearArgs args;
+  memset(&args, 0, sizeof(args));
+  args.bias = (const __half*)bias; args.out = (__half*)out;
+  args.M = (int64_t)b * L; args.N = C; args.K = K; args.ldo = C;
+  args.L = L; args.mt = (L + BM - 1) / BM; args.lkv = lkv;
+  args.scale_log2 = (scale > 0.f ? scale : 1.f / sqrtf((float)HEAD_D)) * 1.4426950408889634f;
+  args.tiles_m = b * args.mt;
+  const int cap = max_ctas > 0 ? max_ctas : sm_count();
+  const int bn = pick_bn_cross(args.tiles_m, C, cap);
+  args.tiles_n = (C + bn - 1) / bn;
+  int ctas = args.tiles_m * args.tiles_n;
+  if (ctas > cap) ctas = cap;
+  CUtensorMap ta, tw, tkv;
+  if (int rc = make_map3d(&ta, x, K, L, b, K, BM)) return rc;
+  if (int rc = make_map2d(&tw, w, C, K, ldw, bn)) return rc;
+  if (int rc = make_map3d(&tkv, kv, 2 * C, lkv, b, ldkv, LKV_ROWS)) return rc;
+  cudaStream_t st = (cudaStream_t)stream;
+  if (bn == 128) return launch_linear<EPI_CROSS, 128>(ta, tw, tkv, args, ctas, st);
+  if (bn == 192) return launch_linear<EPI_CROSS, 192>(ta, tw, tkv, args, ctas, st);
+  return launch_linear<EPI_CROSS, 256>(ta, tw, tkv, args, ctas, st);
 }
 
 namespace {
@@ -394,7 +601,7 @@
         const int q = zc_problem(z, tile);
         const ZeroConvProblem& p = z.p[q];
         const int t = tile - p.tile0;
-        load_tile<BN>(sm, &z.a[q], &z.w[q], t % p.tiles_m, t / p.tiles_m, p.kblocks, stage, phase);
+        load_tile<BN>(sm, &z.a[q], &z.w[q], t % p.tiles_m * BM, -1, t / p.tiles_m, p.kblocks, stage, phase);
       }
     }
   } else {
diff --git a/distrifuser_b200/csrc/tc_ptx.cuh b/distrifuser_b200/csrc/tc_ptx.cuh
--- a/distrifuser_b200/csrc/tc_ptx.cuh
+++ b/distrifuser_b200/csrc/tc_ptx.cuh
@@ -58,6 +58,12 @@
       ::"r"(smem_u32(dst)), "l"((uint64_t)tmap), "r"(smem_u32(bar)), "r"(c0), "r"(c1), "r"(c2), "r"(c3)
       : "memory");
 }
+__device__ __forceinline__ void tma_load_3d(void* dst, const void* tmap, uint64_t* bar, int c0, int c1, int c2) {
+  asm volatile(
+      "cp.async.bulk.tensor.3d.shared::cluster.global.mbarrier::complete_tx::bytes [%0], [%1, {%3, %4, %5}], [%2];"
+      ::"r"(smem_u32(dst)), "l"((uint64_t)tmap), "r"(smem_u32(bar)), "r"(c0), "r"(c1), "r"(c2)
+      : "memory");
+}
 __device__ __forceinline__ void tma_load_2d(void* dst, const void* tmap, uint64_t* bar, int c0, int c1) {
   asm volatile(
       "cp.async.bulk.tensor.2d.shared::cluster.global.mbarrier::complete_tx::bytes [%0], [%1, {%3, %4}], [%2];"
@@ -113,6 +119,14 @@
       : "l"(a_desc), "l"(b_desc), "r"(accumulate));
 }
 
+__device__ __forceinline__ void wgmma_ss_n192(float* d, uint64_t a_desc, uint64_t b_desc, uint32_t accumulate) {
+  asm volatile(
+      "{\n\t.reg .pred p;\n\tsetp.ne.b32 p, %98, 0;\n\t"
+      "wgmma.mma_async.sync.aligned.m64n192k16.f32.f16.f16 {%0, %1, %2, %3, %4, %5, %6, %7, %8, %9, %10, %11, %12, %13, %14, %15, %16, %17, %18, %19, %20, %21, %22, %23, %24, %25, %26, %27, %28, %29, %30, %31, %32, %33, %34, %35, %36, %37, %38, %39, %40, %41, %42, %43, %44, %45, %46, %47, %48, %49, %50, %51, %52, %53, %54, %55, %56, %57, %58, %59, %60, %61, %62, %63, %64, %65, %66, %67, %68, %69, %70, %71, %72, %73, %74, %75, %76, %77, %78, %79, %80, %81, %82, %83, %84, %85, %86, %87, %88, %89, %90, %91, %92, %93, %94, %95}, %96, %97, p, 1, 1, 0, 0;\n\t}"
+      : "+f"(d[0]), "+f"(d[1]), "+f"(d[2]), "+f"(d[3]), "+f"(d[4]), "+f"(d[5]), "+f"(d[6]), "+f"(d[7]), "+f"(d[8]), "+f"(d[9]), "+f"(d[10]), "+f"(d[11]), "+f"(d[12]), "+f"(d[13]), "+f"(d[14]), "+f"(d[15]), "+f"(d[16]), "+f"(d[17]), "+f"(d[18]), "+f"(d[19]), "+f"(d[20]), "+f"(d[21]), "+f"(d[22]), "+f"(d[23]), "+f"(d[24]), "+f"(d[25]), "+f"(d[26]), "+f"(d[27]), "+f"(d[28]), "+f"(d[29]), "+f"(d[30]), "+f"(d[31]), "+f"(d[32]), "+f"(d[33]), "+f"(d[34]), "+f"(d[35]), "+f"(d[36]), "+f"(d[37]), "+f"(d[38]), "+f"(d[39]), "+f"(d[40]), "+f"(d[41]), "+f"(d[42]), "+f"(d[43]), "+f"(d[44]), "+f"(d[45]), "+f"(d[46]), "+f"(d[47]), "+f"(d[48]), "+f"(d[49]), "+f"(d[50]), "+f"(d[51]), "+f"(d[52]), "+f"(d[53]), "+f"(d[54]), "+f"(d[55]), "+f"(d[56]), "+f"(d[57]), "+f"(d[58]), "+f"(d[59]), "+f"(d[60]), "+f"(d[61]), "+f"(d[62]), "+f"(d[63]), "+f"(d[64]), "+f"(d[65]), "+f"(d[66]), "+f"(d[67]), "+f"(d[68]), "+f"(d[69]), "+f"(d[70]), "+f"(d[71]), "+f"(d[72]), "+f"(d[73]), "+f"(d[74]), "+f"(d[75]), "+f"(d[76]), "+f"(d[77]), "+f"(d[78]), "+f"(d[79]), "+f"(d[80]), "+f"(d[81]), "+f"(d[82]), "+f"(d[83]), "+f"(d[84]), "+f"(d[85]), "+f"(d[86]), "+f"(d[87]), "+f"(d[88]), "+f"(d[89]), "+f"(d[90]), "+f"(d[91]), "+f"(d[92]), "+f"(d[93]), "+f"(d[94]), "+f"(d[95])
+      : "l"(a_desc), "l"(b_desc), "r"(accumulate));
+}
+
 __device__ __forceinline__ void wgmma_ss_n256(float* d, uint64_t a_desc, uint64_t b_desc, uint32_t accumulate) {
   asm volatile(
       "{\n\t.reg .pred p;\n\tsetp.ne.b32 p, %130, 0;\n\t"
@@ -129,6 +143,13 @@
       : "r"(a[0]), "r"(a[1]), "r"(a[2]), "r"(a[3]), "l"(b_desc), "r"(accumulate));
 }
 
+__device__ __forceinline__ void wgmma_rs_n80(float* d, const uint32_t* a, uint64_t b_desc, uint32_t accumulate) {
+  asm volatile(
+      "{\n\t.reg .pred p;\n\tsetp.ne.b32 p, %45, 0;\n\t"
+      "wgmma.mma_async.sync.aligned.m64n80k16.f32.f16.f16 {%0, %1, %2, %3, %4, %5, %6, %7, %8, %9, %10, %11, %12, %13, %14, %15, %16, %17, %18, %19, %20, %21, %22, %23, %24, %25, %26, %27, %28, %29, %30, %31, %32, %33, %34, %35, %36, %37, %38, %39}, {%40, %41, %42, %43}, %44, p, 1, 1, 0;\n\t}"
+      : "+f"(d[0]), "+f"(d[1]), "+f"(d[2]), "+f"(d[3]), "+f"(d[4]), "+f"(d[5]), "+f"(d[6]), "+f"(d[7]), "+f"(d[8]), "+f"(d[9]), "+f"(d[10]), "+f"(d[11]), "+f"(d[12]), "+f"(d[13]), "+f"(d[14]), "+f"(d[15]), "+f"(d[16]), "+f"(d[17]), "+f"(d[18]), "+f"(d[19]), "+f"(d[20]), "+f"(d[21]), "+f"(d[22]), "+f"(d[23]), "+f"(d[24]), "+f"(d[25]), "+f"(d[26]), "+f"(d[27]), "+f"(d[28]), "+f"(d[29]), "+f"(d[30]), "+f"(d[31]), "+f"(d[32]), "+f"(d[33]), "+f"(d[34]), "+f"(d[35]), "+f"(d[36]), "+f"(d[37]), "+f"(d[38]), "+f"(d[39])
+      : "r"(a[0]), "r"(a[1]), "r"(a[2]), "r"(a[3]), "l"(b_desc), "r"(accumulate));
+}
 
 __device__ __forceinline__ float ex2(float x) {
   float y;
diff --git a/distrifuser_b200/modules/pp/attn.py b/distrifuser_b200/modules/pp/attn.py
--- a/distrifuser_b200/modules/pp/attn.py
+++ b/distrifuser_b200/modules/pp/attn.py
@@ -90,13 +90,29 @@
         super().__init__(module, distri_config)
         self.kv_cache = None
 
+    def _attend_fused(self, hidden_states, kv):
+        from ... import ops
+        attn = self.module
+        prof = _lib.PROFILE
+        if prof is not None:
+            e0, e1 = torch.cuda.Event(enable_timing=True), torch.cuda.Event(enable_timing=True)
+            e0.record()
+        out = ops.cross_attention(hidden_states, attn.to_q, kv, attn.heads)
+        if prof is not None:
+            e1.record()
+            b, lq, C = out.shape
+            K = hidden_states.shape[-1]
+            prof.append(dict(kernel="linear_kernel", kind="cross", flops=4.0 * b * lq * kv.shape[1] * C,
+                             bytes=2.0 * (b * lq * K + C * K + b * kv.shape[1] * 2 * C + b * lq * C),
+                             shape=(b, lq, kv.shape[1], attn.heads, C // attn.heads), start=e0, end=e1))
+        return out
+
     @nvtx_range("DistriCrossAttentionPP")
     def forward(self, hidden_states, encoder_hidden_states=None, scale: float = 1.0, *args, **kwargs):
         assert encoder_hidden_states is not None
         self._require_cuda_half(hidden_states, "DistriCrossAttentionPP")
         attn = self.module
         from ... import ops
-        q = ops.project("qkv", hidden_states, attn.to_q)
         if self.counter == 0 or self.kv_cache is None:
             kv = self.to_kv(encoder_hidden_states)
             if self.kv_cache is not None and self.kv_cache.shape == kv.shape:
@@ -104,7 +120,11 @@
             else:
                 self.kv_cache = kv
         kv = self.kv_cache
-        out = self._attend(q, kv, [kv.shape[1]], 0, False, kind="cross")
+        if ops.cross_attention_supported(hidden_states, attn.to_q, kv, attn.heads):
+            out = self._attend_fused(hidden_states, kv)
+        else:
+            q = ops.project("qkv", hidden_states, attn.to_q)
+            out = self._attend(q, kv, [kv.shape[1]], 0, False, kind="cross")
         out = self._project_out(out, hidden_states)
         self.counter += 1
         return out
diff --git a/distrifuser_b200/ops.py b/distrifuser_b200/ops.py
--- a/distrifuser_b200/ops.py
+++ b/distrifuser_b200/ops.py
@@ -141,6 +141,32 @@
     return out
 
 
+def cross_attention_supported(x: torch.Tensor, lin: torch.nn.Linear, kv: torch.Tensor, heads: int) -> bool:
+    w = lin.weight
+    if not (x.is_cuda and x.dtype == torch.float16 and w.dtype == torch.float16 and kv.dtype == torch.float16 and
+            x.dim() == 3 and kv.dim() == 3 and kv.shape[0] == x.shape[0] and w.stride(-1) == 1 and kv.stride(-1) == 1 and
+            kv.stride(0) == kv.shape[1] * kv.stride(1) and
+            getattr(lin, "lora_layer", None) is None and (lin.bias is None or lin.bias.dtype == torch.float16)):
+        return False
+    C = w.shape[0]
+    if heads * 64 != C or kv.shape[2] != 2 * C or w.shape[1] != x.shape[-1]:
+        return False
+    return bool(_lib.lib().df_linear_cross_attn_supported(x.shape[0], x.shape[1], C, x.shape[-1], heads, kv.shape[1]))
+
+
+def cross_attention(x: torch.Tensor, lin: torch.nn.Linear, kv: torch.Tensor, heads: int, max_ctas: int = 0) -> torch.Tensor:
+    x = x.contiguous()
+    b, L, K = x.shape
+    w = lin.weight
+    C = w.shape[0]
+    out = torch.empty((b, L, C), dtype=x.dtype, device=x.device)
+    _lib.check(_lib.lib().df_linear_cross_attn_fwd(x.data_ptr(), w.data_ptr(), lin.bias.data_ptr() if lin.bias is not None else None,
+                                                   kv.data_ptr(), out.data_ptr(), b, L, C, K, heads, kv.shape[1], w.stride(0),
+                                                   kv.stride(1), 0.0, max_ctas, torch.cuda.current_stream().cuda_stream),
+               "df_linear_cross_attn_fwd")
+    return out
+
+
 def controlnet_zero_convs(xs, convs, scale: torch.Tensor) -> list[torch.Tensor]:
     import ctypes as C
     n = len(xs)
diff --git a/include/distrifuser_b200.h b/include/distrifuser_b200.h
--- a/include/distrifuser_b200.h
+++ b/include/distrifuser_b200.h
@@ -107,6 +107,10 @@
                   int geglu_block, int publish, int pub_col0, int idx, uint32_t peer_mask, uint64_t tensor_off,
                   uint64_t slot_bytes, int max_ctas, void* stream);
 
+int df_linear_cross_attn_supported(int b, int L, int C, int K, int heads, int lkv);
+int df_linear_cross_attn_fwd(const void* x, const void* w, const void* bias, const void* kv, void* out, int b, int L, int C,
+                             int K, int heads, int lkv, int64_t ldw, int64_t ldkv, float scale, int max_ctas, void* stream);
+
 int df_controlnet_zero_convs(int nproblems, const void* const* x_host, const void* const* w_host, const void* const* bias_host,
                              void* const* out_host, const int64_t* m_host, const int32_t* n_host, const int32_t* k_host,
                              const float* scale, int max_ctas, void* stream);
```

Result: no change. 1507 (median of 6 runs) (-0.9%).
